# DongSky/few-shot-vit

Measured on AMD Instinct MI355X. Metric: episodes_per_sec_5way_5shot_visformer_s, higher is better.
Workload: dtype bf16; 1 GPU; BASELINE configs[1]: Visformer-S (visformer_micro_80) miniImageNet-shaped 5-way 5-shot episodic eval, 15 query/class, 80x80 fp32 NCHW episodes resident in HBM, procedural weights + calibrated BN; images_per_episode=100, encoder_chunk_images=12800, distinct_episode_batches=16, parallelism=episode-parallel x1, one all-reduce of accuracy stats, ranks_seen=1, per_rank_eps=4486.3

## Files before the change

few-shot-vit_amd/_lib.py:

```python
import ctypes as C
import os

_HERE = os.path.dirname(os.path.abspath(__file__))
LIB_PATH = os.path.join(_HERE, 'libfsvit.so')

F32, BF16, F16, BF16X2, F16X2 = 0, 1, 2, 3, 4
ACT_NONE, ACT_GELU, ACT_LRELU = 0, 1, 2
HEAD_COS, HEAD_SQR, HEAD_DOT = 0, 1, 2
ERR_ARG, ERR_KEY, ERR_IMG_SIZE, ERR_WORKSPACE = -1, -2, -3, -4


class Tensor(C.Structure):
    _fields_ = [('name', C.c_char_p), ('data', C.POINTER(C.c_float)), ('ndim', C.c_int),
                ('shape', C.c_int64 * 4)]


class VisformerCfg(C.Structure):
    _fields_ = [('img_size', C.c_int), ('init_channels', C.c_int), ('embed_dim', C.c_int),
                ('depth', C.c_int * 3), ('num_heads', C.c_int), ('mlp_ratio', C.c_float),
                ('group', C.c_int), ('bn_eps', C.c_float)]


class VitCfg(C.Structure):
    _fields_ = [('img_size', C.c_int), ('patch_size', C.c_int), ('embed_dim', C.c_int), ('depth', C.c_int),
                ('num_heads', C.c_int), ('mlp_ratio', C.c_float), ('ln_eps', C.c_float)]


class LvvitCfg(C.Structure):
    _fields_ = [('img_size', C.c_int), ('stem_channels', C.c_int), ('embed_dim', C.c_int), ('depth', C.c_int),
                ('num_heads', C.c_int), ('mlp_ratio', C.c_float), ('skip_lam', C.c_float), ('ln_eps', C.c_float),
                ('bn_eps', C.c_float)]


class ProfRec(C.Structure):
    _fields_ = [('layer', C.c_char * 48), ('kernel_id', C.c_int), ('launches', C.c_int), ('flops', C.c_double),
                ('ms', C.c_double)]


class Param(C.Structure):
    _fields_ = [('name', C.c_char_p), ('data', C.c_void_p), ('grad', C.c_void_p), ('numel', C.c_int64)]


_vp, _fp, _i, _f, _sz = C.c_void_p, C.c_void_p, C.c_int, C.c_float, C.c_size_t
SIGNATURES = {
    'fsvit_last_error': (C.c_char_p, []),
    'fsvit_version': (C.c_char_p, []),
    'fsvit_visformer_create': (_i, [C.POINTER(VisformerCfg), C.POINTER(Tensor), _i, _i, C.POINTER(_vp)]),
    'fsvit_visformer_destroy': (None, [_vp]),
    'fsvit_visformer_out_dim': (_i, [_vp]),
    'fsvit_visformer_dtype': (_i, [_vp]),
    'fsvit_visformer_workspace_bytes': (_sz, [_vp, _i]),
    'fsvit_visformer_forward': (_i, [_vp, _fp, _i, _i, _i, _fp, _vp, _sz, _vp]),
    'fsvit_vit_create': (_i, [C.POINTER(VitCfg), C.POINTER(Tensor), _i, _i, C.POINTER(_vp)]),
    'fsvit_vit_destroy': (None, [_vp]),
    'fsvit_vit_out_dim': (_i, [_vp]),
    'fsvit_vit_workspace_bytes': (_sz, [_vp, _i]),
    'fsvit_vit_forward': (_i, [_vp, _fp, _i, _i, _i, _fp, _vp, _sz, _vp]),
    'fsvit_lvvit_create': (_i, [C.POINTER(LvvitCfg), C.POINTER(Tensor), _i, _i, C.POINTER(_vp)]),
    'fsvit_lvvit_destroy': (None, [_vp]),
    'fsvit_lvvit_out_dim': (_i, [_vp]),
    'fsvit_lvvit_workspace_bytes': (_sz, [_vp, _i]),
    'fsvit_lvvit_forward': (_i, [_vp, _fp, _i, _i, _i, _fp, _vp, _sz, _vp]),
    'fsvit_lvvit_forward_map': (_i, [_vp, _fp, _i, _i, _i, _fp, _fp, _vp, _sz, _vp]),
    'fsvit_stem96_conv': (_i, [_vp, _vp, _fp, _vp, _i, _i, _vp, _i, _i, _i, _i, _i, _vp]),
    'fsvit_encoder_set_tap': (_i, [_vp, C.c_char_p, _vp, _sz]),
    'fsvit_encoder_profile_begin': (_i, [_vp]),
    'fsvit_encoder_profile_end': (_i, [_vp, C.POINTER(ProfRec), _i, C.POINTER(_i)]),
    'fsvit_kernel_name': (C.c_char_p, [_i, _i]),
    'fsvit_proto_head': (_i, [_fp, _fp, _i, _i, _i, _i, _i, _f, _i, _fp, _fp, _fp, _vp]),
    'fsvit_proto_head_devtemp': (_i, [_fp, _fp, _i, _i, _i, _i, _i, _fp, _i, _fp, _fp, _fp, _vp]),
    'fsvit_meta_baseline_forward': (_i, [_vp, _fp, _fp, _i, _i, _i, _i, _i, _i, _f, _i, _fp, _fp, _fp, _fp,
                                         _vp, _sz, _vp]),
    'fsvit_conv_gemm': (_i, [_vp, _vp, _fp, _vp, _fp, _vp] + [_i] * 15 + [_i, _vp]),
    'fsvit_conv_stem_tail': (_i, [_vp, _vp, _fp, _fp, _vp, _i, _i, _vp, _i, _i, _i, _i, _i, _i, _i, _vp]),
    'fsvit_stage1_block': (_i, [_vp, _vp, _vp, _fp, _vp, _vp, _i, _vp]),
    'fsvit_stage1_block_hw': (_i, [_vp, _vp, _vp, _fp, _vp, _vp, _i, _i, _i, _i, _vp]),
    'fsvit_visformer_last_tokens': (_i, [_vp, _vp, _sz, _i, _fp, _vp]),
    'fsvit_visformer_train_tokens': (_i, [_vp, _fp, _vp]),
    'fsvit_visformer_train_set_token_grad': (_i, [_vp, _fp]),
    'fsvit_linear_forward': (_i, [_fp, _fp, _fp, _fp, _i, _i, _i, _vp]),
    'fsvit_linear_backward': (_i, [_fp, _fp, _fp, _fp, _i, _fp, _fp, _i, _i, _i, _vp]),
    'fsvit_token_softlabel': (_i, [_fp, _fp, _i, _i, _i, _i, _i, C.c_double, _vp]),
    'fsvit_soft_target_ce': (_i, [_fp, _fp, _fp, _fp, _i, _i, _f, _vp]),
    'fsvit_row_normalize': (_i, [_fp, _fp, _fp, _i, _i, _vp]),
    'fsvit_row_normalize_backward': (_i, [_fp, _fp, _fp, _fp, _i, _i, _vp]),
    'fsvit_adamw_step': (_i, [_fp, _fp, _fp, _fp, _sz, _f, _f, _f, _f, _f, _i, _vp]),
    'fsvit_adamw_step_multi': (_i, [_vp, _i, _sz, _f, _f, _f, _f, _f, _i, _vp]),
    'fsvit_proj_mlp_rows': (_i, [_vp, _vp, _vp, _vp, _i, _i, _vp, _i, _fp, _vp, _i, _fp, _i, _i, _i, _vp]),
    'fsvit_proj_mlp_rows_dt': (_i, [_vp, _vp, _vp, _vp, _i, _i, _vp, _i, _fp, _vp, _i, _fp, _i, _i, _i, _i, _vp]),
    'fsvit_ln_linear_rows': (_i, [_vp, _vp, _vp, _i, _fp, _i, _i, _i, _f, _vp]),
    'fsvit_ln_linear_rows_dt': (_i, [_vp, _vp, _vp, _i, _fp, _i, _i, _i, _f, _i, _vp]),
    'fsvit_patch_embed2x2': (_i, [_vp, _vp, _vp, _i, _fp, _fp, _i, _i, _i, _i, _vp]),
    'fsvit_patch_embed2x2_dt': (_i, [_vp, _vp, _vp, _i, _fp, _fp, _i, _i, _i, _i, _i, _vp]),
    'fsvit_vit_block_tail': (_i, [_vp, _vp, _vp, _vp, _i, _i, _fp, _vp, _i, _fp, _vp, _i, _fp, _i, _i, _i, _f, _vp]),
    'fsvit_vit_block_tail_dt': (_i, [_vp, _vp, _vp, _vp, _i, _i, _fp, _vp, _i, _fp, _vp, _i, _fp, _i, _i, _i, _f, _i, _vp]),
    'fsvit_mlp_rows': (_i, [_vp, _vp, _vp, _i, _fp, _vp, _i, _fp, _i, _i, _i, _vp]),
    'fsvit_mlp_rows_dt': (_i, [_vp, _vp, _vp, _i, _fp, _vp, _i, _fp, _i, _i, _i, _i, _vp]),
    'fsvit_attention': (_i, [_vp, _vp, _i, _i, _i, _i, _f, _i, _vp]),
    'fsvit_op_attention_route': (_i, [_i, _i, _i]),
    'fsvit_qkv_attention': (_i, [_vp, _vp, _i, _fp, _vp, _i, _i, _i, _i, _i, _f, _vp]),
    'fsvit_qkv_attention_dt': (_i, [_vp, _vp, _i, _fp, _vp, _i, _i, _i, _i, _i, _f, _i, _vp]),
    'fsvit_vit_ln_qkv_attention': (_i, [_vp, _vp, _i, _fp, _vp, _i, _i, _i, _i, _i, _f, _f, _vp]),
    'fsvit_vit_ln_qkv_attention_dt': (_i, [_vp, _vp, _i, _fp, _vp, _i, _i, _i, _i, _i, _f, _f, _i, _vp]),
    'fsvit_im2col27': (_i, [_fp, _vp, _i, _i, _i, _i, _vp]),
    'fsvit_stem_conv1': (_i, [_fp, _vp, _i, _fp, _vp, _vp, _i, _i, _i, _vp]),
    'fsvit_stem_conv1_dt': (_i, [_fp, _vp, _i, _fp, _vp, _vp, _i, _i, _i, _i, _vp]),
    'fsvit_maxpool2_pos': (_i, [_vp, _fp, _vp, _i, _i, _i, _i, _i, _vp]),
    'fsvit_pool_affine': (_i, [_vp, _fp, _fp, _fp, _i, _i, _i, _i, _vp]),
    'fsvit_visformer_trainer_create': (_i, [C.POINTER(VisformerCfg), _i, C.POINTER(_vp)]),
    'fsvit_visformer_trainer_destroy': (None, [_vp]),
    'fsvit_visformer_trainer_workspace_bytes': (_sz, [_vp, C.POINTER(Param), _i, _i, _f]),
    'fsvit_visformer_train_forward': (_i, [_vp, C.POINTER(Param), _i, _fp, _i, _i, _i, _f, _fp, _fp, _vp, _sz, _vp]),
    'fsvit_visformer_train_backward': (_i, [_vp, C.POINTER(Param), _i, _fp, _vp]),
    'fsvit_vit_trainer_create': (_i, [C.POINTER(VitCfg), _i, C.POINTER(_vp)]),
    'fsvit_vit_trainer_destroy': (None, [_vp]),
    'fsvit_vit_trainer_droppath_calls': (_i, [_vp, _f]),
    'fsvit_vit_trainer_workspace_bytes': (_sz, [_vp, C.POINTER(Param), _i, _i, _f]),
    'fsvit_vit_train_forward': (_i, [_vp, C.POINTER(Param), _i, _fp, _i, _i, _i, _f, _fp, _fp, _vp, _sz, _vp]),
    'fsvit_vit_train_backward': (_i, [_vp, C.POINTER(Param), _i, _fp, _vp]),
    'fsvit_lvvit_trainer_create': (_i, [C.POINTER(LvvitCfg), _i, C.POINTER(_vp)]),
    'fsvit_lvvit_trainer_destroy': (None, [_vp]),
    'fsvit_lvvit_trainer_droppath_calls': (_i, [_vp, _f]),
    'fsvit_lvvit_trainer_workspace_bytes': (_sz, [_vp, C.POINTER(Param), _i, _i, _f]),
    'fsvit_lvvit_trainer_set_freeze_bn': (_i, [_vp, _i]),
    'fsvit_lvvit_train_forward': (_i, [_vp, C.POINTER(Param), _i, _fp, _i, _i, _i, _f, _fp, _fp, _vp, _sz, _vp]),
    'fsvit_lvvit_train_backward': (_i, [_vp, C.POINTER(Param), _i, _fp, _vp]),
    'fsvit_lvvit_train_tokens': (_i, [_vp, _fp, _vp]),
    'fsvit_lvvit_train_set_token_grad': (_i, [_vp, _fp]),
    'fsvit_proto_head_backward': (_i, [_fp, _fp, _fp, _i, _i, _i, _i, _i, _f, _fp, _fp, _fp, _vp]),
    'fsvit_proto_head_backward_sqr': (_i, [_fp, _fp, _fp, _i, _i, _i, _i, _i, _f, _fp, _fp, _fp, _vp]),
    'fsvit_proto_head_ce': (_i, [_fp, _fp, _vp, _i, _i, _i, _i, _i, _f, _fp, _i, _fp, _fp, _fp, _fp, _fp, _vp, _vp]),
    'fsvit_proto_head_ce_backward': (_i, [_fp, _fp, _fp, _fp, _i, _i, _i, _i, _i, _f, _fp, _i, _fp, _fp, _fp, _vp, _vp]),
    'fsvit_proto_head_backward_devtemp': (_i, [_fp, _fp, _fp, _i, _i, _i, _i, _i, _fp, _i, _fp, _fp, _fp, _vp]),
    'fsvit_visformer_trainer_set_freeze_bn': (_i, [_vp, _i]),
    'fsvit_sgd_step_multi': (_i, [_vp, _i, _sz, _f, _f, _f, _i, _vp]),
    'fsvit_sgd_step': (_i, [_fp, _fp, _fp, _sz, _f, _f, _f, _i, _vp]),
    'fsvit_sgd_nesterov_step_multi': (_i, [_vp, _i, _sz, _f, _f, _f, _i, _vp]),
    'fsvit_sgd_nesterov_step': (_i, [_fp, _fp, _fp, _sz, _f, _f, _f, _i, _vp]),
    'fsvit_grad_nan_guard_multi': (_i, [_vp, _i, _sz, _vp, _vp]),
    'fsvit_conv1x1_wgrad': (_i, [_vp, _vp, _fp, _i, _i, _i, _i, _vp]),
    'fsvit_conv3x3_wgrad': (_i, [_vp, _vp, _fp, _i, _i, _i, _i, _i, _i, _i, _vp]),
    'fsvit_gconv3x3': (_i, [_vp, _vp, _i, _vp, _i, _i, _i, _i, _vp]),
    'fsvit_image_transform_gather': (_i, [_vp, _i, _i, _vp, _i, _vp, _vp, _vp, _i, _vp, _vp, _vp, _i, _i, _i, _i, _i,
                                          C.POINTER(C.c_float), C.POINTER(C.c_float), _fp, _vp]),
    'fsvit_image_transform_rrc_gather': (_i, [_vp, _i, _i, _vp, _i, _vp, _vp, _i, _i, C.POINTER(C.c_float), C.POINTER(C.c_float), _fp, _vp]),
    'fsvit_image_transform_rrc_u8': (_i, [_vp, _i, _i, _vp, _i, _vp, _vp, _i, _i, _i, _vp, _vp]),
    'fsvit_image_strong_weak': (_i, [_vp, _i, _i, _i, _vp, _i, C.POINTER(C.c_float), C.POINTER(C.c_float), C.c_uint64, _fp, _fp, _vp]),
    'fsvit_image_rand_augment': (_i, [_vp, _i, _i, _i, _vp, _i, _vp, _i, C.POINTER(C.c_uint8), _vp]),
    'fsvit_attention_backward': (_i, [_vp, _vp, _vp, _i, _i, _i, _i, _i, _f, _i, _vp]),
    'fsvit_op_attention_bwd_route': (_i, [_i, _i, _i, _i]),
    'fsvit_op_bn_reduce_blocks': (_i, [_i]),
    'fsvit_op_ln_bwd_blocks': (_i, [_i]),
    'fsvit_op_pool_bn_bwd_blocks': (_i, [_i, _i, _i, _i, _i]),
    'fsvit_op_bn_train_forward': (_i, [_vp, _i, _i, _i, _fp, _fp, _fp, _fp, _f, _f, _i, _vp, _vp, _fp, _i, _vp, _i, _vp, _fp, _fp, _vp]),
    'fsvit_op_bn_train_backward': (_i, [_vp, _vp, _fp, _fp, _fp, _i, _i, _i, _i, _fp, _fp, _vp, _fp, _vp, _i, _vp, _fp, _fp, _fp, _fp, _vp]),
    'fsvit_op_bn_act_bwd': (_i, [_vp, _vp, _fp, _fp, _vp, _vp, _i, _i, _i, _vp]),
    'fsvit_op_stem_tail_train_forward': (_i, [_vp, _fp, _fp, _vp, _fp, _fp, _fp, _vp, _vp, _i, _i, _i, _i, _i, _vp]),
    'fsvit_op_stem_tail_train_backward': (_i, [_vp, _vp, _vp, _vp, _fp, _fp, _fp, _fp, _vp, _vp, _fp, _fp, _fp, _fp, _fp, _fp, _i, _i, _i, _i, _i, _i, _vp]),
    'fsvit_op_pool_act_bwd': (_i, [_vp, _vp, _vp, _i, _i, _i, _i, _i, _vp]),
    'fsvit_op_maxpool2_idx': (_i, [_vp, _fp, _vp, _vp, _i, _i, _i, _i, _i, _vp]),
    'fsvit_op_maxpool2_bwd': (_i, [_vp, _vp, _vp, _i, _i, _i, _i, _i, _vp]),
    'fsvit_op_ln_train_forward': (_i, [_vp, _fp, _fp, _vp, _fp, _fp, _i, _i, _f, _i, _vp]),
    'fsvit_op_ln_train_backward': (_i, [_vp, _vp, _fp, _fp, _fp, _vp, _vp, _fp, _fp, _fp, _i, _i, _i, _vp]),
    'fsvit_op_vit_assemble': (_i, [_vp, _fp, _fp, _vp, _i, _i, _i, _i, _vp]),
    'fsvit_op_vit_patch_rows': (_i, [_vp, _vp, _i, _i, _i, _i, _vp]),
    'fsvit_op_vit_cls_ln_forward': (_i, [_vp, _fp, _fp, _fp, _fp, _fp, _i, _i, _i, _f, _i, _vp]),
    'fsvit_op_vit_cls_ln_backward': (_i, [_fp, _vp, _fp, _fp, _fp, _vp, _fp, _fp, _fp, _i, _i, _i, _i, _vp]),
    'fsvit_op_vit_map_ln_forward': (_i, [_vp, _fp, _fp, _fp, _fp, _fp, _i, _i, _i, _f, _i, _vp]),
    'fsvit_op_vit_map_ln_bwd_blocks': (_i, [_i, _i]),
    'fsvit_op_vit_map_ln_backward': (_i, [_fp, _fp, _vp, _fp, _fp, _fp, _fp, _fp, _vp, _fp, _fp, _fp, _i, _i, _i, _i, _vp]),
    'fsvit_op_gelu': (_i, [_vp, _vp, _vp, _sz, _i, _vp]),
    'fsvit_op_add_scaled': (_i, [_vp, _vp, _fp, _vp, _sz, _sz, _i, _vp]),
    'fsvit_op_avgpool_bwd': (_i, [_fp, _vp, _i, _i, _i, _i, _vp]),
    'fsvit_op_batch_sum': (_i, [_vp, _fp, _i, _sz, _i, _vp]),
    'fsvit_op_bcast_add': (_i, [_vp, _fp, _vp, _i, _sz, _i, _vp]),
    'fsvit_op_colsum': (_i, [_vp, _fp, _fp, _i, _i, _i, _vp]),
    'fsvit_op_unpatch2': (_i, [_vp, _vp, _i, _i, _i, _i, _i, _vp]),
    'fsvit_op_droppath_scales': (_i, [_fp, _fp, _i, _i, C.POINTER(C.c_float), _vp]),
    'fsvit_op_fill_f32': (_i, [_fp, _f, _sz, _vp]),
    'fsvit_op_scale_copy': (_i, [_fp, _fp, _sz, _f, _vp]),
    'fsvit_op_fold_prenorm': (_i, [_fp, _fp, _fp, _vp, _fp, _i, _i, _i, _i, _vp]),
    'fsvit_op_pack_weight': (_i, [_fp, _vp] + [_i] * 13 + [_vp]),
    'fsvit_op_pack_weight_multi': (_i, [C.POINTER(_fp), C.POINTER(_vp), C.POINTER(_i), _i, _i, _vp]),
    'fsvit_op_conv_train': (_i, [_vp, _vp, _fp, _vp, _vp, _vp] + [_i] * 15 + [C.POINTER(_i), _vp]),
    'fsvit_op_gconv3x3_train': (_i, [_vp, _vp, _i, _vp, _vp, _vp, _i, _i, _i, _i, _vp]),
    'fsvit_op_stage1_block_train': (_i, [_vp, _vp, _vp, _fp, _vp, _i, _vp, _vp, _vp, _vp, _vp, _vp, _fp, _fp, _fp, _i, _i, _i, _i, _vp]),
    'fsvit_op_stage1_block_dgrad': (_i, [_vp, _vp, _vp, _vp, _i, _vp, _vp, _vp, _vp, _vp, _i, _i, _i, _i, _vp]),
    'fsvit_emd_head_workspace_bytes': (_sz, [_i, _i, _i, _i, _i]),
    'fsvit_emd_head_forward': (_i, [_fp, _fp, _i, _i, _i, _i, _i, _f, _fp, _fp, _vp, _vp, _sz, _vp]),
# ... 47 lines not shown
```

few-shot-vit_amd/csrc/conv3x3_halo.hip:

```cpp
#include <stdlib.h>

#include <type_traits>

#include "conv_gemm.h"
#include "lds_dma.h"

namespace FSVIT_NS {

__device__ __attribute__((aligned(256))) unsigned char g_zero_page_halo[256];
#define HWAIT(vm) asm volatile("s_waitcnt vmcnt(" #vm ") lgkmcnt(0)" ::: "memory")

template <int CTRL>
__device__ __forceinline__ float quad_xor(float v) {
  return __builtin_bit_cast(float, __builtin_amdgcn_update_dpp(0, __builtin_bit_cast(int, v), CTRL, 0xf, 0xf, true));
}

namespace halo {
constexpr int TR = 8, TW = 40;
constexpr int HR = TR + 2, HP = 44;
constexpr int PLANE = 7168;
constexpr int NPIECE = 7;
constexpr int HBUF = 8 * PLANE;
constexpr int NST = 3, STAGE = 16384;
constexpr int OFF_W = 2 * HBUF;
constexpr int LDS_BYTES = OFF_W + NST * STAGE;
static_assert(LDS_BYTES == 160 * 1024, "the two halo buffers and the weight ring fill the LDS exactly");
}

template <int CIN, bool FUSE_TAIL, bool STATS = false, int CREAL = CIN>
__global__ __launch_bounds__(512, 2) void conv3x3_halo_kernel(const ConvGemmParams p, const int n_tiles) {
  using namespace halo;
  extern __shared__ __attribute__((aligned(16))) unsigned char smem[];
  constexpr int NH = CIN / 64;
  constexpr int NKM = 9 * NH, NKT = NKM + (FUSE_TAIL ? 1 : 0);
  constexpr int MT = 5, NT = 4;
  const int t = threadIdx.x, lane = t & 63;
  const int wave = __builtin_amdgcn_readfirstlane(t >> 6);
  const int wm = wave >> 1, wn = wave & 1;
  const int lrow = lane & 15, lq = lane >> 4;
  const unsigned lds0 = lds_addr(smem);
  unsigned char* const wst0 = smem + OFF_W;

  const unsigned char* const Xb = reinterpret_cast<const unsigned char*>(p.x);
  const unsigned char* const Wb = reinterpret_cast<const unsigned char*>(p.w);
  bf16* __restrict__ Y = reinterpret_cast<bf16*>(p.y);
  const int tiles_per_img = p.H / TR;

  const int fr = ((lrow >> 3) & 1) * 2 + ((lrow >> 1) & 1), fc = ((lrow >> 2) & 1) * 2 + (lrow & 1);
  auto blk_r = [&](int i) { return (wm * MT + i) / (TW / 4); };
  auto blk_c = [&](int i) { return (wm * MT + i) % (TW / 4); };
  f32x4 st0[STATS ? NT : 1], st1[STATS ? NT : 1];
#pragma unroll
  for (int j = 0; j < (STATS ? NT : 1); ++j) st0[j] = st1[j] = f32x4{0.f, 0.f, 0.f, 0.f};
  unsigned xb[MT];
#pragma unroll
  for (int i = 0; i < MT; ++i) xb[i] = (unsigned)(((blk_r(i) * 4 + fr) * HP + blk_c(i) * 4 + fc) * 16 + lq * PLANE);
  const int srow = lane >> 3;
  const unsigned schunk = (unsigned)(((lane & 7) ^ srow) << 4);
  unsigned offB[2];
#pragma unroll
  for (int j = 0; j < 2; ++j) {
    const int R = (2 * wave + j) * 8 + srow;
    const int ch = (R & ~31) + 8 * ((R & 15) >> 2) + 4 * ((R >> 4) & 1) + (R & 3);
    offB[j] = (unsigned)ch * (unsigned)(p.Kw * 2) + schunk;
  }
  const unsigned b_rd = (unsigned)((wn * 64 + lrow) * 128);
  const unsigned sw0 = (unsigned)((lq ^ (lrow & 7)) << 4), sw1 = (unsigned)(((4 + lq) ^ (lrow & 7)) << 4);

  auto issue_w = [&](int wk, int stage) {
    const unsigned d = lds0 + OFF_W + stage * STAGE;
    dma2(offB[0], offB[1], Wb + (size_t)wk * 128, d + (2 * wave) * 1024, d + (2 * wave + 1) * 1024);
  };
  const int x_rs = p.x_planar ? (CIN / 8) * p.W * 16 : p.W * CREAL * 2, x_ps = p.x_planar ? 16 : CREAL * 2;
  auto issue_piece = [&](int j, int lane_o, const unsigned char* base, bool top, bool bot, int nb) {
    const int s = j * 64 + lane_o, hr = s / HP, hc = s - hr * HP;
    const bool ok = (base != nullptr) & (s < HR * HP) & (hc >= 1) & (hc <= TW) & !(top & (hr == 0)) & !(bot & (hr == HR - 1));
    const unsigned long a = (unsigned long)base + (unsigned long)(unsigned)(hr * x_rs + (hc - 1) * x_ps);
    const unsigned long z = (unsigned long)g_zero_page_halo;
    dma1_lane(reinterpret_cast<const void*>(ok ? a : z), lds0 + nb * HBUF + wave * PLANE + j * 1024);
  };
  auto halo_base = [&](int tile, int h) {
    const int bb = tile / tiles_per_img, rr = (tile - bb * tiles_per_img) * TR;
    if constexpr (CREAL != CIN) {
      if (h * 64 + wave * 8 >= CREAL) return (const unsigned char*)nullptr;
    }
    return Xb + (long)(bb * p.H + rr - 1) * x_rs + (p.x_planar ? (h * 8 + wave) * p.W * 16 : h * 128 + wave * 16);
  };

  f32x4 acc[MT][NT];
#pragma unroll
  for (int i = 0; i < MT; ++i)
#pragma unroll
    for (int j = 0; j < NT; ++j) acc[i][j] = f32x4{0.f, 0.f, 0.f, 0.f};

  int tix = blockIdx.x;
  if (tix >= n_tiles) return;
  const int my_tiles = (n_tiles - tix + (int)gridDim.x - 1) / (int)gridDim.x;
  int steps_left = my_tiles * NKT;

  auto wk_of = [&](int q) { return q >= NKM ? NKM : (NH == 2 ? (q >= 9 ? (q - 9) * 2 + 1 : q * 2) : q); };

  {
    const int r00 = (tix % tiles_per_img) * TR;
    const unsigned char* b0 = halo_base(tix, 0);
#pragma unroll
    for (int j = 0; j < NPIECE; ++j) issue_piece(j, lane, b0, r00 == 0, r00 + TR == p.H, 0);
  }
  issue_w(wk_of(0), 0);
  issue_w(wk_of(1 % NKT), 1);
  HWAIT(0);
  bar();
  int st_cur = 0, st_pre = 2, q_pre = 2 % NKT;
  int buf = 0;
#define H_STAMP(acc_)

  auto advance = [&]() {
    st_cur = st_cur == NST - 1 ? 0 : st_cur + 1;
    st_pre = st_pre == NST - 1 ? 0 : st_pre + 1;
    q_pre = q_pre == NKT - 1 ? 0 : q_pre + 1;
    --steps_left;
  };

  while (true) {
    const int tnext = tix + (int)gridDim.x;
    const bool has_next = tnext < n_tiles;
    const int b = tix / tiles_per_img, r0 = (tix - b * tiles_per_img) * TR;
    u32x4 xf0[MT], wf0[NT];

#pragma unroll 1
    for (int h = 0; h < NH; ++h) {
      const int n_tix = h + 1 < NH ? tix : (has_next ? tnext : -1), n_h = h + 1 < NH ? h + 1 : 0;
      const unsigned char* nbase = n_tix >= 0 ? halo_base(n_tix, n_h) : nullptr;
      const int n_r0 = n_tix >= 0 ? (n_tix % tiles_per_img) * TR : 0;
      const bool n_top = n_r0 == 0, n_bot = n_r0 + TR == p.H;
      int lane_o = lane;
      asm volatile("" : "+v"(lane_o));
      u32x4 xf1[MT], wf1[NT];
      {
        const unsigned char* wb = wst0 + st_cur * STAGE + b_rd;
#pragma unroll
        for (int j = 0; j < NT; ++j) wf0[j] = *reinterpret_cast<const u32x4*>(wb + j * 2048 + sw0);
#pragma unroll
        for (int i = 0; i < MT; ++i) xf0[i] = *reinterpret_cast<const u32x4*>(smem + xb[i]);
      }
      H_STAMP(ckP);
      static_for<9>([&](auto tapc) {
        constexpr int TAP = decltype(tapc)::value;
        constexpr int TOFF = ((TAP / 3) * HP + TAP % 3) * 16;
        constexpr int TOFF_N = (((TAP + 1) / 3) * HP + (TAP + 1) % 3) * 16;
        const bool pre_w = steps_left > 2;
        if (pre_w) issue_w(wk_of(q_pre), st_pre);
        __builtin_amdgcn_sched_barrier(0);
        {
          const unsigned char* wb = wst0 + st_cur * STAGE + b_rd;
#pragma unroll
          for (int j = 0; j < NT; ++j) wf1[j] = *reinterpret_cast<const u32x4*>(wb + j * 2048 + sw1);
#pragma unroll
          for (int i = 0; i < MT; ++i) xf1[i] = *reinterpret_cast<const u32x4*>(smem + xb[i] + 4 * PLANE + TOFF);
        }
#pragma unroll
        for (int i = 0; i < MT; ++i)
#pragma unroll
          for (int j = 0; j < NT; ++j) acc[i][j] = mma_chunk<bf16>(wf0[j], xf0[i], acc[i][j]);
#pragma unroll
        for (int k = 0; k < MT + NT; ++k) {
          __builtin_amdgcn_sched_group_barrier(0x008, 1, 0);
          __builtin_amdgcn_sched_group_barrier(0x100, 1, 0);
        }
        __builtin_amdgcn_sched_group_barrier(0x008, MT * NT - (MT + NT), 0);
        __builtin_amdgcn_sched_barrier(0);
        H_STAMP(ckA);
        if (TAP >= 1 && TAP <= NPIECE) { if (pre_w) HWAIT(3); else HWAIT(1); }
        else { if (pre_w) HWAIT(2); else HWAIT(0); }
        H_STAMP(ckV);
        bar();
        H_STAMP(ckW);
        if constexpr (TAP < NPIECE) issue_piece(TAP, lane_o, nbase, n_top, n_bot, buf ^ 1);
        const int st_next = st_cur == NST - 1 ? 0 : st_cur + 1;
        if constexpr (TAP < 8) {
          const unsigned char* wb = wst0 + st_next * STAGE + b_rd;
#pragma unroll
          for (int j = 0; j < NT; ++j) wf0[j] = *reinterpret_cast<const u32x4*>(wb + j * 2048 + sw0);
#pragma unroll
          for (int i = 0; i < MT; ++i) xf0[i] = *reinterpret_cast<const u32x4*>(smem + xb[i] + TOFF_N);
        } else if (FUSE_TAIL) {
          if (h == NH - 1) {
            const bf16* X2 = reinterpret_cast<const bf16*>(p.x2);
#pragma unroll
            for (int i = 0; i < MT; ++i) {
              const int lr = lane_o & 15;
              const int fr_o = ((lr >> 3) & 1) * 2 + ((lr >> 1) & 1), fc_o = ((lr >> 2) & 1) * 2 + (lr & 1);
              const size_t pix = (size_t)(b * p.H + r0 + blk_r(i) * 4 + fr_o) * p.W + blk_c(i) * 4 + fc_o;
              xf0[i] = gload16(X2 + pix * p.x2_cstride + lq * 8);
            }
          }
        }
#pragma unroll
        for (int i = 0; i < MT; ++i)
#pragma unroll
          for (int j = 0; j < NT; ++j) acc[i][j] = mma_chunk<bf16>(wf1[j], xf1[i], acc[i][j]);
        if constexpr (TAP < NPIECE) {
#pragma unroll
          for (int k = 0; k < 8; ++k) {
            __builtin_amdgcn_sched_group_barrier(0x008, 1, 0);
            __builtin_amdgcn_sched_group_barrier(0x002, 3, 0);
          }
#pragma unroll
// ... 98 lines not shown
                  if (posrow && n < CREAL) v[u] += *reinterpret_cast<const f32x4*>(posrow + n + 4 * u);
                } else v[u] += *reinterpret_cast<const f32x4*>(posrow + n + 4 * u);
              }
            }
            bool nst = true;
            if constexpr (CREAL != CIN) nst = n < CREAL;
            if (nst && (!FUSE_TAIL || (lrow_e & 3) == 0)) {
              const bf16x8 o = {(bf16)v[0][0], (bf16)v[0][1], (bf16)v[0][2], (bf16)v[0][3], (bf16)v[1][0], (bf16)v[1][1], (bf16)v[1][2], (bf16)v[1][3]};
              if (!FUSE_TAIL && p.y_planar) *reinterpret_cast<bf16x8*>(Y + (((size_t)(b * p.H + r0 + prow_i) * (p.y_cstride >> 3) + (n >> 3)) * p.W + pcol_i) * 8) = o;
              else *reinterpret_cast<bf16x8*>(Y + orow * p.y_cstride + n) = o;
            }
          }
        }
      };
      auto finish_pooled = [&](auto actf) {
        const int u_e = lrow_e & 3;
        const int nq = wn * 64 + (u_e >> 1) * 32 + lq_e * 8 + (u_e & 1) * 4;
        bool qok = true;
        if constexpr (CREAL != CIN) qok = nq < CREAL;
        const f32x4 bq = (p.bias && qok) ? *reinterpret_cast<const f32x4*>(p.bias + nq) : f32x4{0.f, 0.f, 0.f, 0.f};
        const int ph = p.H >> 1, pw = p.W >> 1;
#pragma unroll
        for (int i = 0; i < MT; ++i) {
          const int py = (r0 + blk_r(i) * 4 + fr_e) >> 1, px = (blk_c(i) * 4 + fc_e) >> 1;
          f32x4 pq;
          if constexpr (CREAL != CIN) pq = (p.pos && qok) ? *reinterpret_cast<const f32x4*>(p.pos + (size_t)(py * pw + px) * p.y_cstride + nq) : f32x4{0.f, 0.f, 0.f, 0.f};
          else pq = *reinterpret_cast<const f32x4*>(p.pos + (size_t)(py * pw + px) * p.y_cstride + nq);
          f32x4 m[NT];
#pragma unroll
          for (int j = 0; j < NT; ++j) {
            m[j] = acc[i][j];
            acc[i][j] = f32x4{0.f, 0.f, 0.f, 0.f};
#pragma unroll
            for (int e = 0; e < 4; ++e) {
              m[j][e] = fmaxf(m[j][e], quad_xor<0xB1>(m[j][e]));
              m[j][e] = fmaxf(m[j][e], quad_xor<0x4E>(m[j][e]));
            }
          }
          f32x4 v = u_e == 0 ? m[0] : (u_e == 1 ? m[1] : (u_e == 2 ? m[2] : m[3]));
          v += bq;
#pragma unroll
          for (int e = 0; e < 4; ++e) v[e] = actf(v[e]);
          v += pq;
          if (qok) store4<bf16>(Y + ((size_t)(b * ph + py) * pw + px) * p.y_cstride + nq, v);
        }
      };
      if (FUSE_TAIL && p.act == ACT_LRELU) finish_pooled([](float x) { return fmaxf(x, 0.1f * x); });
      else if (FUSE_TAIL && p.act == ACT_NONE) finish_pooled([](float x) { return x; });
      else if (p.act == ACT_GELU) finish([](float x) { return gelu_sig(x); });
      else if (p.act == ACT_LRELU) finish([](float x) { return fmaxf(x, 0.1f * x); });
      else finish([](float x) { return x; });
    }
    H_STAMP(ckE);
    if (!has_next) break;
    tix = tnext;
  }
  asm volatile("s_waitcnt vmcnt(0)" ::: "memory");
  if constexpr (STATS) {
    __syncthreads();
    float* red = reinterpret_cast<float*>(smem);
#pragma unroll
    for (int j = 0; j < NT; ++j)
#pragma unroll
      for (int e = 0; e < 4; ++e) {
        float a = st0[j][e], q = st1[j][e];
#pragma unroll
        for (int o = 1; o < 16; o <<= 1) { a += __shfl_xor(a, o); q += __shfl_xor(q, o); }
        if (lrow == 0) {
          const int cl = (j >> 1) * 32 + lq * 8 + (j & 1) * 4 + e;
          red[(wave * 2 + 0) * 64 + cl] = a;
          red[(wave * 2 + 1) * 64 + cl] = q;
        }
      }
    __syncthreads();
    if (t < 256) {
      const int which = t >> 7, c = t & 127, h = c >> 6, cl = c & 63;
      float a = 0.f;
#pragma unroll
      for (int m = 0; m < 4; ++m) a += red[((m * 2 + h) * 2 + which) * 64 + cl];
      p.stats[((size_t)blockIdx.x * 2 + which) * p.y_cstride + c] = a;
    }
  }
}

bool conv3x3_halo_eligible(const ConvGemmParams& p, int dtype) {
  if (dtype != 1) return false;
  if (p.KH != 3 || p.KW != 3 || p.stride != 1 || p.pad != 1 || p.groups != 1) return false;
  if (p.w_cpad) {
    if (p.w_cpad != 128 || p.Cin != 96 || p.N != 96 || p.x_cstride != 96 || p.y_cstride != 96 || p.K != 9 * 96) return false;
    if (p.W != halo::TW || (p.H % halo::TR) || p.OH != p.H || p.OW != p.W) return false;
    if (p.res || p.y2 || p.act == ACT_MUL || p.act == ACT_GELU || p.y_rpi || p.out_f32 || p.w_rstride || p.w_gstride || p.stats || p.x_planar || p.y_planar) return false;
    if (p.pool2) return p.x2 && p.K2 == 32 && p.x2_cstride >= 32 && p.Kw == 9 * 128 + 64;
    return !p.x2 && !p.pos && p.Kw == 9 * 128;
  }
  if (p.N != 128 || p.y_cstride != 128 || p.W != halo::TW || (p.H % halo::TR) || p.OH != p.H || p.OW != p.W) return false;
  if (p.res || p.y2 || p.act == ACT_MUL || p.y_rpi || p.out_f32 || p.w_rstride || p.w_gstride) return false;
  if (p.Cin != p.x_cstride || p.K != 9 * p.Cin) return false;
  if (p.stats && (p.pool2 || p.act != ACT_NONE)) return false;
  if (p.y_planar && (p.pool2 || p.stats)) return false;
  if (p.pool2) return p.Cin == 128 && p.x2 && p.K2 == 32 && p.x2_cstride >= 32 && p.pos && p.Kw == p.K + 64;
  return (p.Cin == 64 || p.Cin == 128) && !p.x2 && !p.pos && p.Kw == p.K;
}

static inline int halo_grid(const ConvGemmParams& p) { const int n_tiles = p.B * (p.H / halo::TR); return n_tiles < 256 ? n_tiles : 256; }
int conv3x3_halo_stats_rows(const ConvGemmParams& p, int dtype) {
  ConvGemmParams q = p;
  float dummy;
  q.stats = &dummy;
  return conv3x3_halo_eligible(q, dtype) ? halo_grid(p) : 0;
}

template <int CIN, bool FUSE_TAIL, bool STATS = false, int CREAL = CIN>
static int launch_halo_t(const ConvGemmParams& p, hipStream_t stream) {
  const int n_tiles = p.B * (p.H / halo::TR);
  auto kern = conv3x3_halo_kernel<CIN, FUSE_TAIL, STATS, CREAL>;
  hipError_t e = hipFuncSetAttribute((const void*)kern, hipFuncAttributeMaxDynamicSharedMemorySize, halo::LDS_BYTES);
  if (e != hipSuccess) return (int)e;
  const int grid = n_tiles < 256 ? n_tiles : 256;
  hipLaunchKernelGGL(kern, dim3(grid), dim3(512), halo::LDS_BYTES, stream, p, n_tiles);
  return (int)hipGetLastError();
}

int launch_conv3x3_halo(const ConvGemmParams& p, hipStream_t stream) {
  if (p.w_cpad) return p.pool2 ? launch_halo_t<128, true, false, 96>(p, stream) : launch_halo_t<128, false, false, 96>(p, stream);
  if (p.pool2) return launch_halo_t<128, true>(p, stream);
  if (p.stats) return p.Cin == 64 ? launch_halo_t<64, false, true>(p, stream) : launch_halo_t<128, false, true>(p, stream);
  return p.Cin == 64 ? launch_halo_t<64, false>(p, stream) : launch_halo_t<128, false>(p, stream);
}

}
```

few-shot-vit_amd/csrc/engine.hip:

```cpp
#include "../../include/fsvit.h"

#include <hip/hip_runtime.h>

#include <cmath>
#include <cstdarg>
#include <cstdio>
#include <cstring>
#include <cstdlib>
#include <utility>
#include <cstdint>
#include <initializer_list>
#include <map>
#include <string>
#include <vector>

#include "kernels.h"
#include "train_kernels.h"

using namespace fsvit;

#define K(fn) ((kdt == FSVIT_F16 || kdt == FSVIT_F16X2) ? fsvit_f16::fn : fsvit::fn)
static inline bool is_x2(int dtype) { return dtype == FSVIT_BF16X2 || dtype == FSVIT_F16X2; }
static inline bool known_dtype(int dtype) { return dtype >= FSVIT_F32 && dtype <= FSVIT_F16X2; }
static inline int kd(int dtype) { return (dtype == FSVIT_F32 || is_x2(dtype)) ? 0 : 1; }
// ... 226 lines not shown
  }
  for (int y = 0; y < k; ++y) for (int x = 0; x < k; ++x) f[(size_t)y * k + x] = f1[y] * f1[x];
  return f;
}

inline double gelu_exact(double z) { return 0.5 * z * (1.0 + std::erf(z * 0.7071067811865476)); }

void gauss_moments_gelu(double mu, double sig, double* mean, double* var) {
  double sw = 0, s1 = 0, s2 = 0;
  for (int j = 0; j <= 256; ++j) {
    const double z = -8.0 + j / 16.0, w = std::exp(-0.5 * z * z), v = gelu_exact(mu + sig * z);
    sw += w; s1 += w * v; s2 += w * v * v;
  }
  *mean = s1 / sw;
  *var = std::max(0.0, s2 / sw - (s1 / sw) * (s1 / sw));
}

double lrelu_mean(double mu, double sig) {
  if (sig <= 0) return mu > 0 ? mu : 0.1 * mu;
  const double t = mu / sig;
  return mu * (0.1 + 0.9 * 0.5 * (1.0 + std::erf(t * 0.7071067811865476))) + 0.9 * sig * std::exp(-0.5 * t * t) * 0.3989422804014327;
}

int pack_layer(EngineBase* h, Layer* L, const float* W, int O, int Ig, int KH, int KW, int groups,
               const std::vector<double>* out_scale, const std::vector<double>* in_scale,
               const std::vector<double>& bias, bool has_bias,
               const std::vector<int>* rowmap, int Npad, const std::vector<int>* colmap, int Kpad,
               const WRound* wr = nullptr, const std::vector<double>* in_mean = nullptr, const double* tapf = nullptr,
               bool use_cst = false, std::vector<double>* corr_out = nullptr) {
  const int bke = 128 / h->es;
  const int N = (rowmap ? Npad : O) / groups;
  const int K = colmap ? Kpad : KH * KW * Ig;
  const int Kw = round_up(K, bke);
  const bool fix = wr && wr->on && in_mean && in_mean->size() >= (size_t)groups * Ig;
  const bool cst = wr && wr->on && use_cst && wr->cst.size() >= (size_t)groups * Ig;
  if (corr_out) corr_out->assign(O, 0.0);
  std::vector<float> pk((size_t)groups * N * Kw, 0.0f);
  std::vector<float> pb((size_t)groups * N, 0.0f);
  for (int o = 0; o < O; ++o) {
    const int row = rowmap ? (*rowmap)[o] : o;
    const double so = out_scale ? (*out_scale)[o] : 1.0;
    const int g0 = (o / (O / groups)) * Ig;
    double corr = 0.0, wc = 0.0;
    for (int c = 0; c < Ig; ++c) {
      const double si = in_scale ? (*in_scale)[c] : 1.0;
      for (int ky = 0; ky < KH; ++ky)
        for (int kx = 0; kx < KW; ++kx) {
          int k = (ky * KW + kx) * Ig + c;
          if (colmap) k = (*colmap)[k];
          const double v = (double)W[(((size_t)o * Ig + c) * KH + ky) * KW + kx] * so * si;
          pk[(size_t)row * Kw + k] = (float)v;
          if (fix) corr -= (wr->rounded(v) - v) * (tapf ? tapf[ky * KW + kx] : 1.0) * (*in_mean)[g0 + c];
          if (cst) wc += v * wr->cst[g0 + c];
        }
    }
    if (has_bias) pb[row] = (float)(bias[o] + corr + wc);
    else if (corr_out) (*corr_out)[o] = corr;
  }
  L->N = N; L->K = K; L->Kw = Kw; L->groups = groups;
  RC_TRY(upload(h, pk, true, &L->w));
  if (has_bias) { void* b; RC_TRY(upload(h, pb, false, &b)); L->bias = (float*)b; }
  return 0;
}

std::vector<double> prenorm_bias(const float* W, int O, int C, const std::vector<double>& t) {
  std::vector<double> b(O, 0.0);
  for (int o = 0; o < O; ++o) {
    double s = 0.0;
    for (int c = 0; c < C; ++c) s += (double)W[(size_t)o * C + c] * t[c];
    b[o] = s;
  }
  return b;
}

int pack_pos(EngineBase* h, const float* pos, int C, int HW, float** out) {
  std::vector<float> p((size_t)HW * C);
  for (int c = 0; c < C; ++c)
    for (int i = 0; i < HW; ++i) p[(size_t)i * C + c] = pos[(size_t)c * HW + i];
  void* d; RC_TRY(upload(h, p, false, &d));
  *out = (float*)d;
  return 0;
}

int build(fsvit_visformer* h, const SD& sd) {
  const int kdt = h->dtype;
  const fsvit_visformer_cfg& cf = h->cfg;
  const double eps = cf.bn_eps;
  const int epc = 16 / h->es;
  const int D = cf.embed_dim;
  h->C0 = cf.init_channels; h->C1 = D / 2; h->C2 = D; h->C3 = h->out_dim = D * 2;
  if (cf.img_size % 16 != 0) return fail(FSVIT_ERR_ARG, "img_size %d must be a multiple of 16", cf.img_size);
  h->H0 = cf.img_size / 2; h->H1 = cf.img_size / 4; h->H2 = cf.img_size / 8; h->H3 = cf.img_size / 16;
  if (cf.group < 2) return fail(FSVIT_ERR_ARG, "group < 2 ('net' setting, visformer.py:137-138) is not supported");
  h->hid1 = h->C1 * 2;
  h->hid2 = (int)(h->C2 * cf.mlp_ratio);
  h->hid3 = (int)(h->C3 * cf.mlp_ratio);
  h->hd2 = (int)std::lround((double)(h->C2 / cf.num_heads));
  h->hd3 = (int)std::lround((double)(h->C3 / cf.num_heads));
  h->hdp2 = K(attention_padded_head_dim)(h->hd2, h->H2 * h->H2, kd(kdt));
  h->hdp3 = K(attention_padded_head_dim)(h->hd3, h->H3 * h->H3, kd(kdt));
  const int Cg = h->hid1 / cf.group;
  if (h->C0 % epc || h->C1 % epc || h->hid1 % cf.group || Cg % epc)
    return fail(FSVIT_ERR_ARG, "channel counts must be multiples of %d for 16-byte K chunks", epc);
  if (!is_pow2(h->C0) || !is_pow2(h->C1) || !is_pow2(h->C2) || !is_pow2(Cg))
    return fail(FSVIT_ERR_ARG, "multi-tap conv input channels must be powers of two");
  if (h->H2 * h->H2 > 128) return fail(FSVIT_ERR_ARG, "attention supports at most 128 tokens (img_size <= 88)");

  std::vector<double> nob;
  WRound wr;
  const char* wr_env = getenv("FSVIT_WROUND");
  wr.on = (kdt == FSVIT_BF16 || kdt == FSVIT_F16) && !(wr_env && wr_env[0] == '0');
  wr.f16 = kdt == FSVIT_F16;
  if (wr.on) wr.cst.assign(h->C1, 0.0);
  auto vec = [&](const std::string& name, int C, bool absolute) {
    const float* p = sd.get(name, {C});
    std::vector<double> v(C, 0.0);
    for (int c = 0; p && c < C; ++c) v[c] = absolute ? std::fabs((double)p[c]) : (double)p[c];
    return v;
  };
  {
    const float* w1 = sd.get("stem.conv1.weight", {h->C0, 3, 3, 3});
    const float* wd = sd.get("stem.downsample.0.weight", {h->C1, 3, 3, 3});
    const float* w2 = sd.get("stem.conv2.weight", {h->C1, h->C0, 3, 3});
    const float* w3 = sd.get("stem.conv3.weight", {h->C1, h->C1, 3, 3});
    Affine b1 = bn_affine(sd, "stem.bn1", h->C0, eps), b2 = bn_affine(sd, "stem.bn2", h->C1, eps);
    Affine b3 = bn_affine(sd, "stem.bn3", h->C1, eps), bd = bn_affine(sd, "stem.downsample.1", h->C1, eps);
    if (!w1 || !wd || !w2 || !w3 || !b1.ok || !b2.ok || !b3.ok || !bd.ok) return FSVIT_ERR_KEY;
    std::vector<int> cm(27);
    for (int k = 0; k < 27; ++k) cm[k] = k;
    std::vector<double> m2(h->C0), m3(h->C1);
    {
      const std::vector<double> be1 = vec("stem.bn1.bias", h->C0, false), ga1 = vec("stem.bn1.weight", h->C0, true);
      const std::vector<double> be2 = vec("stem.bn2.bias", h->C1, false), ga2 = vec("stem.bn2.weight", h->C1, true);
      for (int c = 0; c < h->C0; ++c) m2[c] = lrelu_mean(be1[c], ga1[c]);
      for (int c = 0; c < h->C1; ++c) m3[c] = lrelu_mean(be2[c], ga2[c]);
    }
    const std::vector<double> tf0 = tap_fraction(h->H0, 1, 3, 1);
    RC_TRY(pack_layer(h, &h->conv1, w1, h->C0, 3, 3, 3, 1, &b1.s, nullptr, b1.t, true, nullptr, 0, &cm, 32));
    RC_TRY(pack_layer(h, &h->conv2, w2, h->C1, h->C0, 3, 3, 1, &b2.s, nullptr, b2.t, true, nullptr, 0, nullptr, 0, &wr, &m2, tf0.data()));
    {
      const int bke = 128 / h->es, K = 9 * h->C1, Kmain = round_up(K, bke), Kw = Kmain + bke;
      std::vector<float> pk((size_t)h->C1 * Kw, 0.0f), pb(h->C1);
      for (int o = 0; o < h->C1; ++o) {
        double corr = 0.0;
        for (int c = 0; c < h->C1; ++c)
          for (int t9 = 0; t9 < 9; ++t9) {
            const double v = (double)w3[((size_t)o * h->C1 + c) * 9 + t9] * b3.s[o];
            pk[(size_t)o * Kw + t9 * h->C1 + c] = (float)v;
            if (wr.on) corr -= (wr.rounded(v) - v) * tf0[t9] * m3[c];
          }
        for (int c = 0; c < 3; ++c)
          for (int t9 = 0; t9 < 9; ++t9)
            pk[(size_t)o * Kw + Kmain + t9 * 3 + c] = (float)((double)wd[((size_t)o * 3 + c) * 9 + t9] * bd.s[o]);
        pb[o] = (float)(b3.t[o] + bd.t[o] + corr);
      }
      h->conv3f.N = h->C1; h->conv3f.K = K; h->conv3f.Kw = Kw; h->conv3f.groups = 1;
      RC_TRY(upload(h, pk, true, &h->conv3f.w));
      void* bdev; RC_TRY(upload(h, pb, false, &bdev)); h->conv3f.bias = (float*)bdev;
    }
  }
  {
    const float* p1 = sd.get("pos_embed1", {1, h->C1, h->H1, h->H1});
    const float* p2 = sd.get("pos_embed2", {1, h->C2, h->H2, h->H2});
    const float* p3 = sd.get("pos_embed3", {1, h->C3, h->H3, h->H3});
    if (!p1 || !p2 || !p3) return FSVIT_ERR_KEY;
    RC_TRY(pack_pos(h, p1, h->C1, h->H1 * h->H1, &h->pos1));
    RC_TRY(pack_pos(h, p2, h->C2, h->H2 * h->H2, &h->pos2));
    RC_TRY(pack_pos(h, p3, h->C3, h->H3 * h->H3, &h->pos3));
  }
  std::vector<double> x_mean(h->C1, 0.0);
  h->s1.resize(cf.depth[0]);
  for (int i = 0; i < cf.depth[0]; ++i) {
    const std::string p = "stage1." + std::to_string(i) + ".";
    Affine n2 = bn_affine(sd, p + "norm2.bn", h->C1, eps);
    const float* w1 = sd.get(p + "mlp.conv1.weight", {h->hid1, h->C1, 1, 1});
    const float* w2 = sd.get(p + "mlp.conv2.weight", {h->hid1, Cg, 3, 3});
    const float* w3 = sd.get(p + "mlp.conv3.weight", {h->C1, h->hid1, 1, 1});
    if (!n2.ok || !w1 || !w2 || !w3) return FSVIT_ERR_KEY;
    const std::vector<double> rm = vec(p + "norm2.bn.running_mean", h->C1, false);
    std::vector<double> mh2(h->hid1, 0.0), corr3;
    if (wr.on) {
      if (wr.cst.empty()) wr.cst.assign(h->C1, 0.0);
      const std::vector<double> be = vec(p + "norm2.bn.bias", h->C1, false), ga = vec(p + "norm2.bn.weight", h->C1, true);
      const std::vector<double> tf1 = tap_fraction(h->H1, 1, 3, 1);
      std::vector<double> mh1(h->hid1), vh1(h->hid1);
      for (int n = 0; n < h->hid1; ++n) {
        double mu = 0, var = 0;
        for (int c = 0; c < h->C1; ++c) { const double w = w1[(size_t)n * h->C1 + c]; mu += w * be[c]; var += w * w * ga[c] * ga[c]; }
        gauss_moments_gelu(mu, std::sqrt(var), &mh1[n], &vh1[n]);
// ... 63 lines not shown
    blocks.resize(cf.depth[s - 1]);
    std::vector<int> rowmap(3 * heads * hd), colmap(heads * hd);
    for (int x = 0; x < 3; ++x)
      for (int y = 0; y < heads; ++y)
        for (int z = 0; z < hd; ++z) rowmap[(x * heads + y) * hd + z] = (x * heads + y) * hdp + z;
    for (int y = 0; y < heads; ++y)
      for (int z = 0; z < hd; ++z) colmap[y * hd + z] = y * hdp + z;
    for (int i = 0; i < cf.depth[s - 1]; ++i) {
      const std::string p = "stage" + std::to_string(s) + "." + std::to_string(i) + ".";
      Affine n1 = bn_affine(sd, p + "norm1.bn", C, eps), n2 = bn_affine(sd, p + "norm2.bn", C, eps);
      const float* wq = sd.get(p + "attn.qkv.weight", {3 * heads * hd, C, 1, 1});
      const float* wp = sd.get(p + "attn.proj.weight", {C, heads * hd, 1, 1});
      const float* w1 = sd.get(p + "mlp.conv1.weight", {hid, C, 1, 1});
      const float* w3 = sd.get(p + "mlp.conv3.weight", {C, hid, 1, 1});
      if (!n1.ok || !n2.ok || !wq || !wp || !w1 || !w3) return FSVIT_ERR_KEY;
      const std::vector<double> rm1 = vec(p + "norm1.bn.running_mean", C, false), rm2 = vec(p + "norm2.bn.running_mean", C, false);
      std::vector<double> mctx(heads * hd, 0.0), mh(hid, 0.0), corr_p, corr_3;
      if (wr.on) {
        const std::vector<double> be1 = vec(p + "norm1.bn.bias", C, false);
        const std::vector<double> be2 = vec(p + "norm2.bn.bias", C, false), ga2 = vec(p + "norm2.bn.weight", C, true);
        for (int n = 0; n < heads * hd; ++n) {
          double a = 0;
          for (int c = 0; c < C; ++c) a += (double)wq[((size_t)2 * heads * hd + n) * C + c] * be1[c];
          mctx[n] = a;
        }
        for (int n = 0; n < hid; ++n) {
          double mu = 0, var = 0, dummy;
          for (int c = 0; c < C; ++c) { const double w = w1[(size_t)n * C + c]; mu += w * be2[c]; var += w * w * ga2[c] * ga2[c]; }
          gauss_moments_gelu(mu, std::sqrt(var), &mh[n], &dummy);
        }
      }
      RC_TRY(pack_layer(h, &blocks[i].qkv, wq, 3 * heads * hd, C, 1, 1, 1, nullptr, &n1.s, prenorm_bias(wq, 3 * heads * hd, C, n1.t), true, &rowmap, 3 * heads * hdp, nullptr, 0,
                        &wr, &rm1, nullptr, true));
      RC_TRY(pack_layer(h, &blocks[i].proj, wp, C, heads * hd, 1, 1, 1, nullptr, nullptr, nob, false, nullptr, 0, &colmap, heads * hdp, &wr, &mctx, nullptr, false, &corr_p));
      if (wr.on) for (int o = 0; o < C; ++o) wr.cst[o] += corr_p[o];
      RC_TRY(pack_layer(h, &blocks[i].fc1, w1, hid, C, 1, 1, 1, nullptr, &n2.s, prenorm_bias(w1, hid, C, n2.t), true, nullptr, 0, nullptr, 0, &wr, &rm2, nullptr, true));
      RC_TRY(pack_layer(h, &blocks[i].fc2, w3, C, hid, 1, 1, 1, nullptr, nullptr, nob, false, nullptr, 0, nullptr, 0, &wr, &mh, nullptr, false, &corr_3));
      if (wr.on) {
        x_mean.assign(C, 0.0);
        for (int o = 0; o < C; ++o) {
          double a = rm2[o];
          for (int c = 0; c < hid; ++c) a += (double)w3[(size_t)o * hid + c] * mh[c];
          x_mean[o] = a;
          wr.cst[o] += corr_3[o];
        }
      }
      if (K(mlp_rows_supported)(kd(kdt), C, hid)) {
        const int kc = K(mlp_rows_proj_supported)(C, hid, heads * hdp) ? heads * hdp : 0;
        BlockA& b = blocks[i];
        void* b1i = nullptr;
        RC_TRY(packed_image(h, K(mlp_rows_image_bytes)(C, hid, kc), &b.mlp_img, [&](void* img) {
          HIP_TRY(hipMalloc(&b1i, (size_t)hid * 4));
          h->allocs.push_back(b1i);
          return K(launch_mlp_pack)(b.fc1.w, b.fc1.Kw, b.fc1.bias, b.fc2.w, b.fc2.Kw, b.proj.w, b.proj.Kw, kc, img, (float*)b1i, C, hid, nullptr);
        }));
        b.mlp_b1 = (float*)b1i;
        b.mlp_kc = kc;
      }
      if (K(qkv_attn_supported)(kd(kdt), C, heads, hdp, (s == 2 ? h->H2 : h->H3) * (s == 2 ? h->H2 : h->H3))) {
        RC_TRY(packed_image(h, K(qkv_attn_image_bytes)(), &blocks[i].qa_img,
                            [&](void* img) { return K(launch_qkv_attn_pack)(blocks[i].qkv.w, blocks[i].qkv.Kw, img, nullptr); }));
      } else if (K(qkv_attn_rows_supported)(kd(kdt), C, heads, hdp, (s == 2 ? h->H2 : h->H3) * (s == 2 ? h->H2 : h->H3))) {
        RC_TRY(packed_image(h, K(ln_gemm_rows_image_bytes)(C, 3 * heads * hdp), &blocks[i].qar_img,
                            [&](void* img) { return K(launch_qkv_attn_rows_pack)(blocks[i].qkv.w, blocks[i].qkv.Kw, img, C, heads, hdp, nullptr); }));
      } else if (K(gemm_rows_supported)(kd(kdt), C, 3 * heads * hdp)) {
        RC_TRY(packed_image(h, K(ln_gemm_rows_image_bytes)(C, 3 * heads * hdp), &blocks[i].qr_img,
                            [&](void* img) { return K(launch_ln_gemm_pack)(blocks[i].qkv.w, blocks[i].qkv.Kw, img, C, 3 * heads * hdp, nullptr); }));
      }
    }
  }
  {
    Affine bn = bn_affine(sd, "norm.bn", h->C3, eps);
    if (!bn.ok) return FSVIT_ERR_KEY;
    std::vector<float> s(h->C3), t(h->C3);
    for (int c = 0; c < h->C3; ++c) { s[c] = (float)bn.s[c]; t[c] = (float)(bn.t[c] + (wr.on ? bn.s[c] * wr.cst[c] : 0.0)); }
    void* d; RC_TRY(upload(h, s, false, &d)); h->fscale = (float*)d;
    RC_TRY(upload(h, t, false, &d)); h->fshift = (float*)d;
  }
  return 0;
}

struct Plan {
  size_t patches, c1, c2;
  size_t ha, hb;
  size_t qkv, ctx, hid;
  size_t x1, x1b, x2, x3;
  size_t total;
};

size_t align256(size_t v) { return (v + 255) / 256 * 256; }

Plan make_plan(const fsvit_visformer* h, size_t Bc) {
  Plan p;
  const size_t es = h->es, P0 = (size_t)h->H0 * h->H0, P1 = (size_t)h->H1 * h->H1, P2 = (size_t)h->H2 * h->H2, P3 = (size_t)h->H3 * h->H3;
  const int heads = h->cfg.num_heads;
  size_t off = 0;
  auto take = [&](size_t bytes) { size_t o = off; off += align256(bytes); return o; };
  p.x1 = take(Bc * P1 * h->C1 * es);
  p.x1b = take(Bc * P1 * h->C1 * es);
  p.x2 = take(Bc * P2 * h->C2 * es);
  p.x3 = take(Bc * P3 * h->C3 * es);
  const size_t scratch0 = off;
  p.patches = take(Bc * P0 * 32 * es);
  p.c1 = take(Bc * P0 * h->C0 * es);
  p.c2 = take(Bc * P0 * h->C1 * es);
  size_t hi = off;
  off = scratch0;
  p.ha = take(Bc * P1 * h->hid1 * es);
  p.hb = take(Bc * P1 * h->hid1 * es);
  if (off > hi) hi = off;
  off = scratch0;
  size_t q2 = Bc * P2 * 3 * heads * h->hdp2 * es, q3 = Bc * P3 * 3 * heads * h->hdp3 * es;
  size_t c2 = Bc * P2 * heads * h->hdp2 * es, c3 = Bc * P3 * heads * h->hdp3 * es;
  size_t h2 = Bc * P2 * h->hid2 * es, h3 = Bc * P3 * h->hid3 * es;
  p.qkv = take(q2 > q3 ? q2 : q3);
  p.ctx = take(c2 > c3 ? c2 : c3);
  p.hid = take(h2 > h3 ? h2 : h3);
  if (off > hi) hi = off;
  p.total = hi;
  return p;
}

ConvGemmParams conv_params(const Layer& L, const void* x, void* y, int B, int H, int W, int Cin, int x_cstride,
                           int KH, int KW, int stride, int pad, int y_cstride, int act,
                           const void* res, int res_first, const float* pos) {
  ConvGemmParams p;
  p.x = x; p.w = L.w; p.bias = L.bias; p.res = res; p.pos = pos; p.y = y;
  p.B = B; p.H = H; p.W = W; p.Cin = Cin; p.x_cstride = x_cstride;
  p.OH = (H + 2 * pad - KH) / stride + 1; p.OW = (W + 2 * pad - KW) / stride + 1;
  p.KH = KH; p.KW = KW; p.stride = stride; p.pad = pad;
  p.N = L.N; p.y_cstride = y_cstride; p.K = L.K; p.Kw = L.Kw; p.M = B * p.OH * p.OW;
  p.groups = L.groups; p.act = act; p.res_first = res_first; p.log2Cin = ilog2(Cin);
  p.x2 = nullptr; p.x2_cstride = 0; p.K2 = 0; p.pool2 = 0; p.y_rpi = 0; p.y_row0 = 0;
  p.w_gstride = 0; p.w_rstride = 0; p.out_f32 = 0; p.y2 = nullptr; p.stats = nullptr;
  return p;
}

int tap(EngineBase* h, const std::string& name, const void* src, size_t bytes, bool first, hipStream_t st) {
  if (!first || h->taps.empty()) return 0;
  auto it = h->taps.find(name);
  if (it == h->taps.end() || it->second.dst == nullptr) return 0;
  size_t n = bytes < it->second.bytes ? bytes : it->second.bytes;
  HIP_TRY(hipMemcpyAsync(it->second.dst, src, n, hipMemcpyDeviceToDevice, st));
  return 0;
}

enum { KID_GEMM256 = 0, KID_GEMM64 = 1, KID_GEMM32 = 2, KID_IM2COL = 3, KID_MAXPOOL = 4, KID_ATTN = 5, KID_POOL = 6, KID_HEAD = 7, KID_STAGE1 = 8, KID_GEMM128 = 9, KID_HALO = 12, KID_MLPROWS = 13, KID_QKVATTN = 15, KID_STEMCONV1 = 16, KID_GCONV_X2 = 14, KID_STAGE1RING = 17, KID_LNGEMM = 18, KID_QKVATTNROWS = 19, KID_VITATTNROWS = 20 };


template <typename F>
int timed(EngineBase* h, hipStream_t st, const char* layer, int kernel, double flops, F&& launch) {
  if (!h->profiling) return launch();
  hipEvent_t e0 = h->prof_last, e1;
  if (!e0) { HIP_TRY(hipEventCreate(&e0)); HIP_TRY(hipEventRecord(e0, st)); }
  int rc = launch();
  if (rc != 0) return rc;
  HIP_TRY(hipEventCreate(&e1));
  HIP_TRY(hipEventRecord(e1, st));
  h->prof.push_back(ProfEntry{layer, kernel, flops, e0, e1});
  h->prof_last = e1;
  return 0;
}

static constexpr int stem_slice_images() { return 3200; }

int run_gemm(EngineBase* h, hipStream_t st, const char* layer, const Layer& L, const ConvGemmParams& p, double n_true, double k_true) {
  const int kdt = h->dtype;
  const double flops = 2.0 * (double)p.M * n_true * k_true * (double)p.groups;
  static const int kid_of_cfg[4] = {KID_GEMM256, KID_GEMM64, KID_GEMM32, KID_GEMM128};
  const int route = K(conv_gemm_route)(p, kg(kdt));
  const int kid = route == 0 ? KID_HALO : route == 1 ? KID_GEMM256 : route == 3 ? KID_GCONV_X2 : kid_of_cfg[K(conv_gemm_v2_config)(p)];
  return timed(h, st, layer, kid, flops, [&]() { return K(launch_conv_gemm)(p, kg(kdt), st); });
}

int forward_chunk(fsvit_visformer* h, const float* x, int Bc, float* feat, unsigned char* ws, bool first, hipStream_t st,
                  const float* xsrc2 = nullptr, int B1 = 0) {
  const Plan pl = make_plan(h, Bc);
  const int kdt = h->dtype, dt = kd(kdt);
  const size_t es = h->es;
  const int heads = h->cfg.num_heads;
  void *patches = ws + pl.patches, *c1 = ws + pl.c1, *c2 = ws + pl.c2;
  void *x1 = ws + pl.x1, *x1b = ws + pl.x1b, *x2 = ws + pl.x2, *x3 = ws + pl.x3, *ha = ws + pl.ha, *hb = ws + pl.hb;
  void *qkv = ws + pl.qkv, *ctx = ws + pl.ctx, *hid = ws + pl.hid;
  const int img = h->cfg.img_size;

  h->prof_last = nullptr;
  if (!xsrc2) B1 = Bc;
  const bool conv1_fused = K(stem_conv1_supported)(dt, img, h->C0);
  ConvGemmParams p2 = conv_params(h->conv2, c1, c2, Bc, h->H0, h->H0, h->C0, h->C0, 3, 3, 1, 1, h->C1, ACT_LRELU, nullptr, 0, nullptr);
  ConvGemmParams p3 = conv_params(h->conv3f, c2, x1, Bc, h->H0, h->H0, h->C1, h->C1, 3, 3, 1, 1, h->C1, ACT_LRELU, nullptr, 0, h->pos1);
  p3.x2 = patches; p3.x2_cstride = 32; p3.K2 = 32; p3.pool2 = 1;
  const bool planar = conv1_fused && K(conv_gemm_route)(p2, kg(kdt)) == 0 && K(conv_gemm_route)(p3, kg(kdt)) == 0;
  p2.x_planar = p2.y_planar = p3.x_planar = planar ? 1 : 0;
  if (planar) {
    const int S = stem_slice_images();
    const size_t s_pat = (size_t)h->H0 * h->H0 * 32 * es, s_c1 = (size_t)h->H0 * h->H0 * h->C0 * es, s_c2 = (size_t)h->H0 * h->H0 * h->C1 * es,
                 s_x1 = (size_t)h->H1 * h->H1 * h->C1 * es;
    const double fl1 = 2.0 * 27.0 * h->C0 * h->H0 * h->H0;
    for (int g0 = 0; g0 < Bc; g0 += S) {
      const int g1 = g0 + S < Bc ? g0 + S : Bc;
      for (int part = 0; part < 2; ++part) {
        const int a = part == 0 ? g0 : (g0 > B1 ? g0 : B1), b = part == 0 ? (g1 < B1 ? g1 : B1) : g1;
        if (a >= b) continue;
        const float* src = part == 0 ? x + (size_t)a * 3 * img * img : xsrc2 + (size_t)(a - B1) * 3 * img * img;
        RC_TRY(timed(h, st, "stem.im2col+conv1", KID_STEMCONV1, fl1 * (b - a), [&]() {
          return K(launch_stem_conv1)(src, (unsigned char*)patches + a * s_pat, (unsigned char*)c1 + a * s_c1, h->conv1.w, h->conv1.Kw, h->conv1.bias, b - a, st, 1); }));
      }
      ConvGemmParams q2 = p2, q3 = p3;
      q2.x = (const unsigned char*)c1 + g0 * s_c1; q2.y = (unsigned char*)c2 + g0 * s_c2; q2.B = g1 - g0; q2.M = (g1 - g0) * q2.OH * q2.OW;
      q3.x = (const unsigned char*)c2 + g0 * s_c2; q3.x2 = (const unsigned char*)patches + g0 * s_pat; q3.y = (unsigned char*)x1 + g0 * s_x1;
      q3.B = g1 - g0; q3.M = (g1 - g0) * q3.OH * q3.OW;
      RC_TRY(run_gemm(h, st, "stem.conv2", h->conv2, q2, h->C1, 9.0 * h->C0));
      RC_TRY(run_gemm(h, st, "stem.conv3+down+pool", h->conv3f, q3, h->C1, 9.0 * h->C1 + 27.0));
    }
  } else {
    if (conv1_fused) {
      const double fl1 = 2.0 * 27.0 * h->C0 * h->H0 * h->H0;
      RC_TRY(timed(h, st, "stem.im2col+conv1", KID_STEMCONV1, fl1 * B1, [&]() {
        return K(launch_stem_conv1)(x, patches, c1, h->conv1.w, h->conv1.Kw, h->conv1.bias, B1, st, 0); }));
      if (Bc > B1)
        RC_TRY(timed(h, st, "stem.im2col+conv1", KID_STEMCONV1, fl1 * (Bc - B1), [&]() {
          return K(launch_stem_conv1)(xsrc2, (unsigned char*)patches + (size_t)B1 * h->H0 * h->H0 * 32 * es, (unsigned char*)c1 + (size_t)B1 * h->H0 * h->H0 * h->C0 * es,
                                   h->conv1.w, h->conv1.Kw, h->conv1.bias, Bc - B1, st, 0); }));
    } else {
      RC_TRY(timed(h, st, "stem.im2col", KID_IM2COL, 0.0, [&]() { return K(launch_im2col27)(x, patches, B1, img, img, h->H0, h->H0, dt, st); }));
      if (Bc > B1)
        RC_TRY(timed(h, st, "stem.im2col", KID_IM2COL, 0.0, [&]() {
          return K(launch_im2col27)(xsrc2, (unsigned char*)patches + (size_t)B1 * h->H0 * h->H0 * 32 * es, Bc - B1, img, img, h->H0, h->H0, dt, st); }));
      RC_TRY(run_gemm(h, st, "stem.conv1", h->conv1, conv_params(h->conv1, patches, c1, Bc, h->H0, h->H0, 32, 32, 1, 1, 1, 0, h->C0, ACT_LRELU, nullptr, 0, nullptr), h->C0, 27));
    }
    RC_TRY(run_gemm(h, st, "stem.conv2", h->conv2, p2, h->C1, 9.0 * h->C0));
    RC_TRY(run_gemm(h, st, "stem.conv3+down+pool", h->conv3f, p3, h->C1, 9.0 * h->C1 + 27.0));
  }
  RC_TRY(tap(h, "stem", x1, (size_t)Bc * h->H1 * h->H1 * h->C1 * es, first, st));

  const int Cg = h->hid1 / h->cfg.group;
  const bool fuse1 = K(stage1_ring_supported)(dt, h->C1, h->hid1, h->cfg.group, h->H1) && h->s1.size() && h->s1[0].c2.Kw == 320;
  for (size_t i = 0; i < h->s1.size(); ++i) {
    const Block1& b = h->s1[i];
    if (fuse1) {
      const double fl = 2.0 * Bc * h->H1 * h->H1 * ((double)h->hid1 * h->C1 + (double)h->hid1 * 9 * Cg + (double)h->C1 * h->hid1);
      RC_TRY(timed(h, st, "stage1.block", KID_STAGE1RING, fl,
                   [&]() { return K(launch_stage1_ring)(x1, x1b, b.c1.w, b.c1.bias, b.c2.w, b.c3.w, Bc, h->H1, h->H1, st, b.c3s); }));
      std::swap(x1, x1b);
    } else {
      RC_TRY(run_gemm(h, st, "stage1.mlp.conv1", b.c1, conv_params(b.c1, x1, ha, Bc, h->H1, h->H1, h->C1, h->C1, 1, 1, 1, 0, h->hid1, ACT_GELU, nullptr, 0, nullptr), h->hid1, h->C1));
      RC_TRY(run_gemm(h, st, "stage1.mlp.conv2", b.c2, conv_params(b.c2, ha, hb, Bc, h->H1, h->H1, Cg, h->hid1, 3, 3, 1, 1, h->hid1, ACT_GELU, nullptr, 0, nullptr), Cg, 9.0 * Cg));
      RC_TRY(run_gemm(h, st, "stage1.mlp.conv3", b.c3, conv_params(b.c3, hb, x1, Bc, h->H1, h->H1, h->hid1, h->hid1, 1, 1, 1, 0, h->C1, ACT_NONE, x1, 0, nullptr), h->C1, h->hid1));
    }
    RC_TRY(tap(h, "stage1." + std::to_string(i), x1, (size_t)Bc * h->H1 * h->H1 * h->C1 * es, first, st));
  }

  for (int s = 2; s <= 3; ++s) {
    const int Ci = s == 2 ? h->C1 : h->C2, C = s == 2 ? h->C2 : h->C3;
    const int Hi = s == 2 ? h->H1 : h->H2, Ho = s == 2 ? h->H2 : h->H3;
    const int hidc = s == 2 ? h->hid2 : h->hid3, hd = s == 2 ? h->hd2 : h->hd3, hdp = s == 2 ? h->hdp2 : h->hdp3;
    void* xin = s == 2 ? x1 : x2;
    void* xs = s == 2 ? x2 : x3;
    const Layer& pe = s == 2 ? h->pe2 : h->pe3;
    const float* pos = s == 2 ? h->pos2 : h->pos3;
    const size_t xbytes = (size_t)Bc * Ho * Ho * C * es;
    const std::string sp = "stage" + std::to_string(s);
    if (h->pe_img[s - 2]) {
      RC_TRY(timed(h, st, s == 2 ? "patch_embed2" : "patch_embed3", KID_LNGEMM, 2.0 * Bc * Ho * Ho * 4.0 * Ci * C,
                   [&]() { return K(launch_patch_embed_rows)(xin, xs, h->pe_img[s - 2], pe.bias, pos, Bc, Hi, Ci, C, st); }));
    } else
    RC_TRY(run_gemm(h, st, s == 2 ? "patch_embed2" : "patch_embed3", pe, conv_params(pe, xin, xs, Bc, Hi, Hi, Ci, Ci, 2, 2, 2, 0, C, ACT_NONE, nullptr, 0, pos), C, 4.0 * Ci));
    RC_TRY(tap(h, "patch_embed" + std::to_string(s), xs, xbytes, first, st));
    const std::vector<BlockA>& blocks = s == 2 ? h->s2 : h->s3;
    const float scale = 1.0f / std::sqrt((float)hd);
    const int S = Ho * Ho;
    for (size_t i = 0; i < blocks.size(); ++i) {
      const BlockA& b = blocks[i];
      if (b.qa_img) {
        RC_TRY(timed(h, st, (sp + ".attn.qkv+core").c_str(), KID_QKVATTN, 2.0 * Bc * S * (3.0 * heads * hd) * C + 4.0 * Bc * heads * (double)S * S * hd,
                     [&]() { return K(launch_qkv_attn)(xs, ctx, b.qa_img, b.qkv.bias, Bc, S, scale, st); }));
      } else if (b.qar_img) {
        RC_TRY(timed(h, st, (sp + ".attn.qkv+core").c_str(), KID_QKVATTNROWS, 2.0 * Bc * S * (3.0 * heads * hd) * C + 4.0 * Bc * heads * (double)S * S * hd,
                     [&]() { return K(launch_qkv_attn_rows)(xs, ctx, b.qar_img, b.qkv.bias, Bc, S, C, heads, hdp, scale, st); }));
      } else {
      if (b.qr_img) {
        RC_TRY(timed(h, st, (sp + ".attn.qkv").c_str(), KID_LNGEMM, 2.0 * Bc * S * (3.0 * heads * hd) * C,
// ... 17 lines not shown
        RC_TRY(run_gemm(h, st, (sp + ".mlp.conv1").c_str(), b.fc1, conv_params(b.fc1, xs, hid, Bc, Ho, Ho, C, C, 1, 1, 1, 0, hidc, ACT_GELU, nullptr, 0, nullptr), hidc, C));
        RC_TRY(run_gemm(h, st, (sp + ".mlp.conv3").c_str(), b.fc2, conv_params(b.fc2, hid, xs, Bc, Ho, Ho, hidc, hidc, 1, 1, 1, 0, C, ACT_NONE, xs, 0, nullptr), C, hidc));
      }
      RC_TRY(tap(h, sp + "." + std::to_string(i), xs, xbytes, first, st));
    }
  }
  RC_TRY(timed(h, st, "norm.pool", KID_POOL, 0.0, [&]() { return K(launch_pool_affine)(x3, h->fscale, h->fshift, feat, Bc, h->H3 * h->H3, h->C3, dt, st); }));
  return 0;
}

size_t visformer_plan_bytes(const EngineBase* h, size_t Bc) { return make_plan(static_cast<const fsvit_visformer*>(h), Bc).total; }
int visformer_chunk(EngineBase* h, const float* x, int Bc, float* feat, unsigned char* ws, bool first, hipStream_t st) {
  return forward_chunk(static_cast<fsvit_visformer*>(h), x, Bc, feat, ws, first, st);
}

template <class H>
void encoder_destroy(H* h) {
  if (!h) return;
  for (void* p : h->allocs) (void)hipFree(p);
  delete h;
}

template <class H, class Cfg>
int encoder_create(const Cfg* cfg, const fsvit_tensor* state_dict, int n_tensors, int dtype, H** out, bool bad_cfg, const char* bad_cfg_msg, int kind,
                   int (*build_fn)(H*, const SD&), size_t (*plan_bytes)(const EngineBase*, size_t),
                   int (*chunk)(EngineBase*, const float*, int, float*, unsigned char*, bool, hipStream_t), const char* size_fmt) {
  if (!cfg || !state_dict || !out || n_tensors <= 0) return fail(FSVIT_ERR_ARG, "null argument");
  if (!known_dtype(dtype)) return fail(FSVIT_ERR_ARG, "unknown dtype %d", dtype);
  if (bad_cfg) return fail(FSVIT_ERR_ARG, "%s", bad_cfg_msg);
  H* h = new H();
  h->kind = kind;
  h->cfg = *cfg;
  h->img_size = cfg->img_size;
  h->dtype = dtype;
  h->es = storage_bytes(dtype);
  h->plan_bytes = plan_bytes; h->chunk = chunk; h->size_fmt = size_fmt;
  SD sd{state_dict, n_tensors};
  int rc = build_fn(h, sd);
  if (rc != 0) { encoder_destroy(h); return rc; }
  *out = h;
  return 0;
}

size_t encoder_workspace_bytes(const EngineBase* h, int chunk_images) {
  if (!h || chunk_images <= 0) return 0;
  return h->plan_bytes(h, (size_t)chunk_images);
}

const char* const SIZE_FMT_VISFORMER = "Input image size (%d*%d) does not match model (%d*%d).";
const char* const SIZE_FMT_VIT = "Input image size (%d*%d) doesn't match model (%d*%d).";

int encoder_forward(EngineBase* h, const float* x, int n_img, int img_h, int img_w, float* feat, void* ws, size_t ws_bytes, void* stream) {
  if (h && n_img <= 0) return 0;
  if (!h || !x || !feat || !ws) return fail(FSVIT_ERR_ARG, "null argument");
  if (img_h != h->img_size || img_w != h->img_size) return fail(FSVIT_ERR_IMG_SIZE, h->size_fmt, img_h, img_w, h->img_size, h->img_size);
  if (((uintptr_t)ws & 255) != 0) return fail(FSVIT_ERR_ARG, "workspace must be 256-byte aligned");
  int lo = 0, hi = n_img;
  while (lo < hi) {
    int mid = (lo + hi + 1) / 2;
    if (h->plan_bytes(h, (size_t)mid) <= ws_bytes) lo = mid; else hi = mid - 1;
  }
  if (lo < 1) return fail(FSVIT_ERR_WORKSPACE, "workspace of %zu bytes cannot hold one image (need %zu)", ws_bytes, h->plan_bytes(h, 1));
  const size_t img_elems = (size_t)3 * img_h * img_w;
  for (int off = 0; off < n_img; off += lo) {
    const int bc = n_img - off < lo ? n_img - off : lo;
    int rc = h->chunk(h, x + (size_t)off * img_elems, bc, feat + (size_t)off * h->out_dim, (unsigned char*)ws, off == 0, (hipStream_t)stream);
    if (rc != 0) return rc;
  }
  return 0;
}

}

extern "C" int fsvit_visformer_create(const fsvit_visformer_cfg* cfg, const fsvit_tensor* state_dict, int n_tensors,
                                      int dtype, fsvit_visformer** out) {
  const bool bad = cfg && (cfg->num_heads < 1 || cfg->embed_dim < 2 || cfg->init_channels < 1 || cfg->depth[0] < 0 || cfg->depth[1] < 0 || cfg->depth[2] < 0);
  return encoder_create(cfg, state_dict, n_tensors, dtype, out, bad, "bad Visformer configuration", KIND_VISFORMER, build, visformer_plan_bytes, visformer_chunk,
                        SIZE_FMT_VISFORMER);
}
extern "C" void fsvit_visformer_destroy(fsvit_visformer* h) { encoder_destroy(h); }
extern "C" int fsvit_visformer_out_dim(const fsvit_visformer* h) { return h ? h->out_dim : 0; }
extern "C" int fsvit_visformer_dtype(const fsvit_visformer* h) { return h ? h->dtype : -1; }
extern "C" size_t fsvit_visformer_workspace_bytes(const fsvit_visformer* h, int chunk_images) { return encoder_workspace_bytes(h, chunk_images); }

extern "C" int fsvit_encoder_set_tap(void* hv, const char* name, void* dst_dev, size_t bytes) {
  EngineBase* h = static_cast<EngineBase*>(hv);
  if (!h || !name) return fail(FSVIT_ERR_ARG, "null argument");
  if (!dst_dev) h->taps.erase(name);
  else h->taps[name] = Tap{dst_dev, bytes};
  return 0;
}

extern "C" int fsvit_visformer_forward(fsvit_visformer* h, const float* x, int n_img, int img_h, int img_w,
                                       float* feat, void* ws, size_t ws_bytes, void* stream) {
  return encoder_forward(h, x, n_img, img_h, img_w, feat, ws, ws_bytes, stream);
}

extern "C" int fsvit_visformer_last_tokens(fsvit_visformer* h, const void* ws, size_t ws_bytes, int n_img, float* tokens, void* stream) {
  const int kdt = h ? h->dtype : FSVIT_BF16;
  if (!h || !ws || !tokens || n_img <= 0) return fail(FSVIT_ERR_ARG, "bad argument");
  const Plan pl = make_plan(h, (size_t)n_img);
  if (pl.total > ws_bytes) return fail(FSVIT_ERR_WORKSPACE, "last_tokens: the forward of %d images did not fit one chunk of this workspace", n_img);
  RC_TRY(K(launch_tokens_to_f32)((const unsigned char*)ws + pl.x3, h->fscale, h->fshift, tokens, (size_t)n_img * h->H3 * h->H3 * h->C3, h->C3, kd(kdt),
                              (hipStream_t)stream));
  return 0;
}

extern "C" int fsvit_proto_head(const float* fs, const float* fq, int E, int way, int shot, int Q, int D, float temp,
                                int method, float* logits, float* acc, float* loss, void* stream) {
  if (!fs || !fq || !logits) return fail(FSVIT_ERR_ARG, "null argument");
  if (method != FSVIT_HEAD_COS && method != FSVIT_HEAD_SQR && method != FSVIT_HEAD_DOT) return fail(FSVIT_ERR_ARG, "unknown head method %d", method);
  RC_TRY(fsvit::launch_proto_head(fs, fq, E, way, shot, Q, D, temp, method, logits, acc, loss, (hipStream_t)stream, nullptr));
  return 0;
}

extern "C" int fsvit_proto_head_devtemp(const float* fs, const float* fq, int E, int way, int shot, int Q, int D, const float* temp_dev,
                                        int method, float* logits, float* acc, float* loss, void* stream) {
  if (!fs || !fq || !logits || !temp_dev) return fail(FSVIT_ERR_ARG, "null argument");
  if (method != FSVIT_HEAD_COS && method != FSVIT_HEAD_SQR && method != FSVIT_HEAD_DOT) return fail(FSVIT_ERR_ARG, "unknown head method %d", method);
  RC_TRY(fsvit::launch_proto_head(fs, fq, E, way, shot, Q, D, 0.f, method, logits, acc, loss, (hipStream_t)stream, temp_dev));
  return 0;
}

extern "C" int fsvit_meta_baseline_forward(void* hv, const float* x_shot, const float* x_query, int E, int way,
                                           int shot, int Q, int img_h, int img_w, float temp, int method, float* logits,
                                           float* acc, float* loss, float* feat, void* ws, size_t ws_bytes, void* stream) {
  if (!hv || !feat) return fail(FSVIT_ERR_ARG, "null argument");
  EngineBase* eb = static_cast<EngineBase*>(hv);
  if (!eb->chunk) return fail(FSVIT_ERR_ARG, "not an fsvit encoder handle");
  const int ns = E * way * shot, nq = E * Q, D = eb->out_dim;
  {
    if (eb->kind == KIND_VISFORMER && x_shot && x_query && ns > 0 && nq > 0) {
      fsvit_visformer* h = static_cast<fsvit_visformer*>(eb);
      if (img_h != h->cfg.img_size || img_w != h->cfg.img_size)
        return fail(FSVIT_ERR_IMG_SIZE, SIZE_FMT_VISFORMER, img_h, img_w, h->cfg.img_size, h->cfg.img_size);
      if (ws && ((uintptr_t)ws & 255) == 0 && make_plan(h, (size_t)ns + nq).total <= ws_bytes) {
        int rc1 = forward_chunk(h, x_shot, ns + nq, feat, (unsigned char*)ws, true, (hipStream_t)stream, x_query, ns);
        if (rc1 != 0) return rc1;
        return fsvit_proto_head(feat, feat + (size_t)ns * D, E, way, shot, Q, D, temp, method, logits, acc, loss, stream);
      }
    }
  }
  int rc = encoder_forward(eb, x_shot, ns, img_h, img_w, feat, ws, ws_bytes, stream);
  if (rc != 0) return rc;
  rc = encoder_forward(eb, x_query, nq, img_h, img_w, feat + (size_t)ns * D, ws, ws_bytes, stream);
  if (rc != 0) return rc;
  return fsvit_proto_head(feat, feat + (size_t)ns * D, E, way, shot, Q, D, temp, method, logits, acc, loss, stream);
}

extern "C" int fsvit_conv_gemm(const void* x, const void* w, const float* bias, const void* res, const float* pos, void* y,
                               int B, int H, int W, int Cin, int x_cstride, int KH, int KW, int stride, int pad, int N,
                               int y_cstride, int Kw, int groups, int act, int res_first, int dtype, void* stream) {
  const int kdt = dtype;
  if (!known_dtype(dtype)) return fail(FSVIT_ERR_ARG, "unknown dtype %d", dtype);
  if (!x || !w || !y) return fail(FSVIT_ERR_ARG, "null argument");
  const int es = storage_bytes(dtype), epc = 16 / es, bke = 128 / es;
  if (Cin % epc || x_cstride % epc || N % 4 || y_cstride % 4 || Kw % bke || Kw < KH * KW * Cin)
    return fail(FSVIT_ERR_ARG, "conv_gemm alignment: Cin/x_cstride %% %d, N/y_cstride %% 4, Kw %% %d", epc, bke);
  if (KH * KW > 1 && !is_pow2(Cin) && Cin % 32) return fail(FSVIT_ERR_ARG, "multi-tap conv needs a power-of-two Cin or a multiple of 32");
  Layer L; L.w = const_cast<void*>(w); L.bias = const_cast<float*>(bias); L.N = N; L.K = KH * KW * Cin; L.Kw = Kw; L.groups = groups;
  ConvGemmParams p = conv_params(L, x, y, B, H, W, Cin, x_cstride, KH, KW, stride, pad, y_cstride, act, res, res_first, pos);
  RC_TRY(K(launch_conv_gemm)(p, kg(dtype), (hipStream_t)stream));
  return 0;
}

extern "C" int fsvit_conv_stem_tail(const void* x, const void* w, const float* bias, const float* pos, const void* x2, int x2_cstride, int K2,
// ... 234 lines not shown
  void* img = nullptr;
  if (C == 512) {
    if (!K(qkv_attn_rows_supported)(1, C, heads, hdp, S) || kw < C)
      return fail(FSVIT_ERR_ARG, "fsvit_qkv_attention: C = 512 needs head dim 96 (padded) and S <= 32");
    HIP_TRY(hipMalloc(&img, K(ln_gemm_rows_image_bytes)(C, 3 * heads * hdp)));
    int rc = K(launch_qkv_attn_rows_pack)(wqkv, kw, img, C, heads, hdp, st);
    if (rc == 0) rc = K(launch_qkv_attn_rows)(x, ctx, img, bias, B, S, C, heads, hdp, scale, st);
    (void)hipStreamSynchronize(st);
    (void)hipFree(img);
    if (rc != 0) return hipfail((hipError_t)rc, "fsvit_qkv_attention");
    return 0;
  }
  if (!K(qkv_attn_supported)(1, C, heads, hdp, S) || kw < C)
    return fail(FSVIT_ERR_ARG, "fsvit_qkv_attention: only C = 256, 6 heads x 48 (padded), S <= 112 is built");
  HIP_TRY(hipMalloc(&img, K(qkv_attn_image_bytes)()));
  int rc = K(launch_qkv_attn_pack)(wqkv, kw, img, st);
  if (rc == 0) rc = K(launch_qkv_attn)(x, ctx, img, bias, B, S, scale, st);
  (void)hipStreamSynchronize(st);
  (void)hipFree(img);
  if (rc != 0) return hipfail((hipError_t)rc, "fsvit_qkv_attention");
  return 0;
}

extern "C" int fsvit_vit_ln_qkv_attention(const void* x, const void* wqkv, int kw, const float* bias, void* ctx, int B, int S, int C, int heads, int hdp,
                                          float eps, float scale, void* stream) {
  return fsvit_vit_ln_qkv_attention_dt(x, wqkv, kw, bias, ctx, B, S, C, heads, hdp, eps, scale, FSVIT_BF16, stream);
}
extern "C" int fsvit_vit_ln_qkv_attention_dt(const void* x, const void* wqkv, int kw, const float* bias, void* ctx, int B, int S, int C, int heads, int hdp,
                                          float eps, float scale, int dtype, void* stream) {
  const int kdt = dtype;
  if (!half_dtype(dtype)) return fail(FSVIT_ERR_ARG, "fsvit_vit_ln_qkv_attention: 16-bit storage only (bf16 / f16)");
  if (!x || !wqkv || !ctx) return fail(FSVIT_ERR_ARG, "null argument");
  if (!K(vit_attn_rows_supported)(1, C, heads, hdp, S) || kw < C)
    return fail(FSVIT_ERR_ARG, "fsvit_vit_ln_qkv_attention: built for C = 384, head dim 64, S <= 256");
  hipStream_t st = (hipStream_t)stream;
  void* img = nullptr;
  HIP_TRY(hipMalloc(&img, K(ln_gemm_rows_image_bytes)(C, 3 * heads * hdp)));
  int rc = K(launch_qkv_attn_rows_pack)(wqkv, kw, img, C, heads, hdp, st);
  if (rc == 0) rc = K(launch_vit_attn_rows)(x, ctx, img, bias, B, S, C, heads, hdp, eps, scale, st);
  (void)hipStreamSynchronize(st);
  (void)hipFree(img);
  if (rc != 0) return hipfail((hipError_t)rc, "fsvit_vit_ln_qkv_attention");
  return 0;
}

extern "C" int fsvit_op_attention_route(int S, int hdp, int dtype) {
  const int kdt = dtype;
  if (!known_dtype(dtype)) return -1;
  return K(attention_route)(S, hdp, kg(dtype));
}

extern "C" int fsvit_attention(const void* qkv, void* ctx, int B, int S, int heads, int hdp, float scale, int dtype, void* stream) {
  const int kdt = dtype;
  if (!known_dtype(dtype)) return fail(FSVIT_ERR_ARG, "unknown dtype %d", dtype);
  if (!qkv || !ctx) return fail(FSVIT_ERR_ARG, "null argument");
  if (B < 0 || heads < 1) return fail(FSVIT_ERR_ARG, "fsvit_attention: B = %d, heads = %d (B >= 0, heads >= 1)", B, heads);
  if (K(attention_route)(S, hdp, kg(dtype)) < 0)
    return fail(FSVIT_ERR_ARG, "fsvit_attention: no kernel covers S = %d, hdp = %d in dtype %d (fsvit.h)", S, hdp, dtype);
  int rc = K(launch_attention)(qkv, ctx, B, S, heads, hdp, scale, kg(dtype), (hipStream_t)stream);
  if (rc != 0) return hipfail((hipError_t)rc, "attention");
  return 0;
}

extern "C" int fsvit_im2col27(const float* x, void* out, int B, int H, int W, int dtype, void* stream) {
  const int kdt = dtype;
  if (!known_dtype(dtype)) return fail(FSVIT_ERR_ARG, "unknown dtype %d", dtype);
  if (!x || !out || (H & 1) || (W & 1)) return fail(FSVIT_ERR_ARG, "bad argument");
  RC_TRY(K(launch_im2col27)(x, out, B, H, W, H / 2, W / 2, kd(dtype), (hipStream_t)stream));
  return 0;
}

extern "C" int fsvit_stem_conv1(const float* x, const void* w, int kw, const float* bias, void* patches, void* c1, int B, int H, int W, void* stream) {
  return fsvit_stem_conv1_dt(x, w, kw, bias, patches, c1, B, H, W, FSVIT_BF16, stream);
}
extern "C" int fsvit_stem_conv1_dt(const float* x, const void* w, int kw, const float* bias, void* patches, void* c1, int B, int H, int W, int dtype, void* stream) {
  const int kdt = dtype;
  if (!half_dtype(dtype)) return fail(FSVIT_ERR_ARG, "fsvit_stem_conv1: 16-bit storage only (bf16 / f16)");
  if (!x || !w || !patches || !c1 || kw < 32) return fail(FSVIT_ERR_ARG, "bad argument");
  if (H != W || !K(stem_conv1_supported)(1, H, 64)) return fail(FSVIT_ERR_ARG, "fsvit_stem_conv1: only 80x80 images, 64 output channels are built");
  RC_TRY(K(launch_stem_conv1)(x, patches, c1, w, kw, bias, B, (hipStream_t)stream, 0));
  return 0;
}

extern "C" int fsvit_maxpool2_pos(const void* in, const float* pos, void* out, int B, int OH, int OW, int C, int dtype, void* stream) {
  const int kdt = dtype;
  if (!known_dtype(dtype)) return fail(FSVIT_ERR_ARG, "unknown dtype %d", dtype);
  if (!in || !out || C % 4) return fail(FSVIT_ERR_ARG, "bad argument");
  RC_TRY(K(launch_maxpool2_pos)(in, pos, out, B, OH, OW, C, kd(dtype), (hipStream_t)stream));
  return 0;
}

extern "C" int fsvit_pool_affine(const void* x, const float* scale, const float* shift, float* feat, int B, int HW, int C,
                                 int dtype, void* stream) {
  const int kdt = dtype;
  if (!known_dtype(dtype)) return fail(FSVIT_ERR_ARG, "unknown dtype %d", dtype);
  if (!x || !scale || !shift || !feat || C % 4 || C < 4 || HW < 1)
    return fail(FSVIT_ERR_ARG, "fsvit_pool_affine: null argument, C %% 4 != 0 or HW < 1 (the mean over no positions divides by zero)");
  RC_TRY(K(launch_pool_affine)(x, scale, shift, feat, B, HW, C, kd(dtype), (hipStream_t)stream));
  return 0;
}

extern "C" const char* fsvit_kernel_name(int kernel_id, int dtype) {
#define FSVIT_KERNEL_NAMES(T)                                                                                                                              \
  {"gemm256_kernel", "conv_gemm_v2_kernel<" T ",128,64,2,2,3>", "conv_gemm_v2_kernel<" T ",128,32,4,1,3>", "im2col27_kernel<" T ">", "maxpool2_pos_kernel<" T ">", \
   "attention_v2_kernel<" T ",...>", "pool_affine_kernel<" T ">", "proto_head_kernel", "stage1_block_kernel", "conv_gemm_v2_kernel<" T ",128,128,2,2,2>",          \
   "patchify_kernel<" T ">", "layernorm_kernel<" T ">", "conv3x3_halo_kernel", "mlp_rows_kernel", "-", "qkv_attn_kernel", "stem_conv1_kernel",                   \
   "stage1_ring_kernel", "ln_gemm_rows_kernel", "qkv_attn_rows_kernel", "vit_attn_rows_kernel"}
  static const char* const names[3][21] = {FSVIT_KERNEL_NAMES("float"), FSVIT_KERNEL_NAMES("__bf16"), FSVIT_KERNEL_NAMES("_Float16")};
#undef FSVIT_KERNEL_NAMES
  static const char* x2n[] = {"gemm256_x2_kernel", "conv_gemm_v2_kernel<f32x2l,128,64,2,2,3>", "conv_gemm_v2_kernel<f32x2l,128,32,4,1,3>", "", "", "", "", "", "", "conv_gemm_v2_kernel<f32x2l,128,128,2,2,2>"};
  if (kernel_id < 0 || kernel_id > 20) return "?";
  if (kernel_id == KID_STAGE1RING && kd(dtype) == 1) return "stage1_w4_kernel";
  if (is_x2(dtype)) return kernel_id == 14 ? "gconv3x3_x2_kernel" : (kernel_id == 0 || kernel_id == 1 || kernel_id == 2 || kernel_id == 9) ? x2n[kernel_id] : names[0][kernel_id];
  return names[dtype == FSVIT_F32 ? 0 : dtype == FSVIT_F16 ? 2 : 1][kernel_id];
}

extern "C" int fsvit_encoder_profile_begin(void* hv) {
  EngineBase* h = static_cast<EngineBase*>(hv);
  if (!h) return fail(FSVIT_ERR_ARG, "null argument");
  h->prof.clear();
  h->prof_last = nullptr;
  h->profiling = true;
  return 0;
}

extern "C" int fsvit_encoder_profile_end(void* hv, fsvit_prof_rec* out, int max_recs, int* n_out) {
  EngineBase* h = static_cast<EngineBase*>(hv);
  if (!h || !out || !n_out) return fail(FSVIT_ERR_ARG, "null argument");
  h->profiling = false;
  std::vector<fsvit_prof_rec> agg;
  hipEvent_t freed = nullptr;
  for (ProfEntry& e : h->prof) {
    HIP_TRY(hipEventSynchronize(e.e1));
    float ms = 0.f;
    HIP_TRY(hipEventElapsedTime(&ms, e.e0, e.e1));
    size_t k = 0;
    for (; k < agg.size(); ++k)
      if (e.layer == agg[k].layer && e.kernel == agg[k].kernel_id) break;
    if (k == agg.size()) {
      fsvit_prof_rec r;
      memset(&r, 0, sizeof(r));
      snprintf(r.layer, sizeof(r.layer), "%s", e.layer.c_str());
      r.kernel_id = e.kernel;
      agg.push_back(r);
    }
    agg[k].flops += e.flops;
    agg[k].ms += ms;
    agg[k].launches += 1;
  }
  for (ProfEntry& e : h->prof) {
    if (e.e0 != freed) (void)hipEventDestroy(e.e0);
    (void)hipEventDestroy(e.e1);
    freed = e.e1;
  }
  h->prof.clear();
  h->prof_last = nullptr;
  *n_out = (int)agg.size();
  if ((int)agg.size() > max_recs) return fail(FSVIT_ERR_ARG, "profile has %zu records, buffer holds %d", agg.size(), max_recs);
  for (size_t i = 0; i < agg.size(); ++i) out[i] = agg[i];
  return 0;
}

struct VitBlock {
  Layer qkv, proj, fc1, fc2;
  void* mlp_img = nullptr;
  float* mlp_b1 = nullptr;
  void* qkv_img = nullptr;
  void* attn_img = nullptr;
};

struct fsvit_vit : EngineBase {
  fsvit_vit_cfg cfg;
  int D = 0, S = 0, np = 0, npw = 0, Kp = 0, hd = 0, hdp = 0, hid = 0;
  Layer pe;
  float *pos_patch = nullptr;
  float *cls_pos0 = nullptr;
  float *ng = nullptr, *nb = nullptr;
  std::vector<VitBlock> blocks;
};

namespace {

std::vector<double> add_vec(const std::vector<double>& a, const float* b, int n) {
  std::vector<double> r(n);
  for (int i = 0; i < n; ++i) r[i] = a[i] + (double)b[i];
  return r;
}

int pack_vit_blocks(EngineBase* h, const SD& sd, int depth, int D, int heads, int hd, int hdp, int hid, int S, bool qkv_bias, double res_scale,
                    std::vector<VitBlock>* blocks_out) {
  std::vector<VitBlock>& blocks = *blocks_out;
  std::vector<int> rowmap(3 * heads * hd), colmap(heads * hd);
  for (int x = 0; x < 3; ++x)
    for (int y = 0; y < heads; ++y)
// ... 370 lines not shown
```

few-shot-vit_amd/csrc/kernels_decl.inc:

```
namespace FSVIT_DECL_NS {
using namespace fsvit_types;


int launch_im2col27(const float* x_nchw, void* out, int B, int H, int W, int OH, int OW, int dtype, hipStream_t s);
bool stem_conv1_supported(int dtype, int img, int C0);
int launch_stem_conv1(const float* x_nchw, void* patches, void* c1, const void* w, int kw, const float* bias, int B, hipStream_t s, int c1_planar = 0);
int launch_maxpool2_pos(const void* in, const float* pos, void* out, int B, int OH, int OW, int C, int dtype, hipStream_t s);

int launch_attention(const void* qkv, void* ctx, int B, int S, int heads, int hdp, float scale, int dtype, hipStream_t s);
int attention_route(int S, int hdp, int dtype);
size_t attention_lds_bytes(int S, int hdp, int dtype);
int attention_padded_head_dim(int hd, int S, int dtype);

int launch_pool_affine(const void* x, const float* scale, const float* shift, float* feat, int B, int HW, int C, int dtype, hipStream_t s);

bool stage1_ring_supported(int dtype, int C1, int hid, int group, int H1);
int launch_stage1_ring(const void* x, void* y, const void* w1, const float* b1, const void* w2, const void* w3, int B, int H, int W, hipStream_t s, const void* w3s = nullptr);
int launch_stage1_ring16(const void* x, void* y, const void* w1, const float* b1, const void* w2, const void* w3, int B, int H, int W, hipStream_t s);
int launch_stage1_w4(const void* x, void* y, const void* w1, const float* b1, const void* w2, const void* w3, int B, int H, int W, hipStream_t s, const void* w3s = nullptr);
int launch_stage1_w4_prescale(const void* w, void* ws, int n, hipStream_t s);
int launch_stage1_ring_block_train(const void* x, void* out, const void* w1f, const float* b1f, const void* w2, const void* w3, void* h1, void* g1, void* h2, void* g2,
                                   void* xn, const float* sa, const float* sb, const float* scale, float* stats, int B, int H, int W, hipStream_t s);
int launch_stage1_ring_dgrad(const void* dz3, void* dxn, const void* w3t, const void* w2t, const void* w1t, const void* g2, const void* g1, void* dz2, void* dz1,
                             int B, int H, int W, hipStream_t s);

bool mlp_rows_supported(int dtype, int C, int hid);
bool mlp_rows_proj_supported(int C, int hid, int KC);
size_t mlp_rows_image_bytes(int C, int hid, int KC);
int launch_mlp_pack(const void* w1, int k1w, const float* b1, const void* w2, int k2w, const void* wp, int kpw, int KC, void* wimg, float* b1img, int C,
                    int hid, hipStream_t s);
int launch_mlp_rows(const void* x, void* y, const void* wimg, const float* b1img, const float* b2, const void* ctx, int KC, int M, int C, int hid,
                    hipStream_t s);
bool mlp_rows_ln_supported(int dtype, int C, int hid, int KC);
int launch_mlp_rows_ln(const void* x, void* y, const void* wimg, const float* b1img, const float* bproj, const float* b2, const void* ctx, int KC, int M,
                       int C, int hid, float eps, hipStream_t s);

bool ln_gemm_rows_supported(int dtype, int C, int N);
size_t ln_gemm_rows_image_bytes(int C, int N);
int launch_ln_gemm_pack(const void* w, int kw, void* wimg, int C, int N, hipStream_t s);
int launch_ln_gemm_rows(const void* x, void* y, const void* wimg, const float* bias, int M, int C, int N, float eps, hipStream_t s);
bool gemm_rows_supported(int dtype, int C, int N);
int launch_gemm_rows(const void* x, void* y, const void* wimg, const float* bias, int M, int C, int N, hipStream_t s);

bool patch_embed_rows_supported(int dtype, int Ci, int H, int N);
int launch_patch_embed_rows(const void* x, void* y, const void* wimg, const float* bias, const float* pos, int B, int H, int Ci, int N, hipStream_t s);

bool qkv_attn_rows_supported(int dtype, int C, int heads, int hdp, int S);
int launch_qkv_attn_rows_pack(const void* w, int kw, void* wimg, int C, int heads, int hdp, hipStream_t s);
int launch_qkv_attn_rows(const void* x, void* ctx, const void* wimg, const float* bias, int B, int S, int C, int heads, int hdp, float scale, hipStream_t s);
bool vit_attn_rows_supported(int dtype, int C, int heads, int hdp, int S);
int launch_vit_attn_rows(const void* x, void* ctx, const void* wimg, const float* bias, int B, int S, int C, int heads, int hdp, float eps, float scale, hipStream_t s);

bool qkv_attn_supported(int dtype, int C, int heads, int hdp, int S);
size_t qkv_attn_image_bytes();
int launch_qkv_attn_pack(const void* w, int kw, void* img, hipStream_t s);
int launch_qkv_attn(const void* x, void* ctx, const void* wimg, const float* bias, int B, int S, float scale, hipStream_t s);

int launch_tokens_to_f32(const void* in, const float* scale, const float* shift, float* out, size_t n, int C, int dtype, hipStream_t s);
int launch_add_f32_into(void* inout, const float* add, size_t n, int dtype, hipStream_t s);

int launch_patchify(const float* x_nchw, void* out, int B, int img, int p, int Kp, int dtype, hipStream_t s);
int launch_cls_pos(const float* cls_plus_pos0, void* tokens, int B, int S, int D, int dtype, hipStream_t s);
int launch_layernorm(const void* x, void* y, int M, int D, float eps, int dtype, hipStream_t s);
int launch_final_ln_cls(const void* tokens, const float* gamma, const float* beta, float* feat, int B, int S, int D, float eps, int dtype, hipStream_t s);
int launch_final_ln_map(const void* tokens, const float* gamma, const float* beta, float* feat, float* map, int B, int S, int D, float eps, int dtype, hipStream_t s);

bool wgrad3x3_supported(int dtype, int O, int Ig, int groups, int W);
size_t wgrad3x3_scratch_bytes(int O, int Ig, int groups, int M, int dtype = 1);
bool wgrad1x1_supported(int dtype, int N, int C);
int wgrad1x1_splits(int N, int C, int M, int dtype = 1);
int launch_wgrad1x1(const void* x, int xld, int C, const void* dz, int zld, int N, float* y, int M, int Kc_pad, hipStream_t s, int dtype = 1);
bool gconv3x3_supported(int dtype, int O, int Ig, int groups, int KH, int KW, int stride, int pad, int W);
int launch_gconv3x3(const void* x, const void* w_packed, int Kw, void* y, int B, int H, int W, hipStream_t s, void* y2 = nullptr, const void* mul = nullptr);
int launch_wgrad3x3(const void* x, int xld, const void* dz, int zld, float* dw, float* scratch, int B, int H, int W, int O, int Ig, int groups, hipStream_t s,
                    int* defer = nullptr, int dtype = 1);

}
```

few-shot-vit_amd/csrc/stem.hip:

```cpp
#include "fsvit_common.h"
#include "kernels.h"

namespace FSVIT_NS {

template <typename T>
__global__ __launch_bounds__(256) void im2col27_kernel(const float* __restrict__ x, T* __restrict__ out,
                                                       int B, int H, int W, int OH, int OW) {
  const int m = blockIdx.x * 256 + threadIdx.x;
  const int M = B * OH * OW;
  if (m >= M) return;
  const int b = m / (OH * OW);
  const int rem = m - b * OH * OW;
  const int oy = rem / OW, ox = rem - oy * OW;
  const float* xb = x + (size_t)b * 3 * H * W;
  float v[32];
#pragma unroll
  for (int ky = 0; ky < 3; ++ky) {
    const int iy = oy * 2 - 1 + ky;
#pragma unroll
    for (int kx = 0; kx < 3; ++kx) {
      const int ix = ox * 2 - 1 + kx;
      const bool ok = (unsigned)iy < (unsigned)H && (unsigned)ix < (unsigned)W;
#pragma unroll
      for (int c = 0; c < 3; ++c)
        v[(ky * 3 + kx) * 3 + c] = ok ? xb[(size_t)c * H * W + (size_t)iy * W + ix] : 0.0f;
    }
  }
#pragma unroll
  for (int k = 27; k < 32; ++k) v[k] = 0.0f;
  T* o = out + (size_t)m * 32;
#pragma unroll
  for (int k = 0; k < 32; k += 4) store4<T>(o + k, f32x4{v[k], v[k + 1], v[k + 2], v[k + 3]});
}

template <typename T>
__global__ __launch_bounds__(256) void maxpool2_pos_kernel(const T* __restrict__ in, const float* __restrict__ pos,
                                                           T* __restrict__ out, int B, int OH, int OW, int C) {
  const int c4 = C / 4;
  const size_t total = (size_t)B * OH * OW * c4;
  for (size_t idx = (size_t)blockIdx.x * 256 + threadIdx.x; idx < total; idx += (size_t)gridDim.x * 256) {
    const int cq = (int)(idx % c4);
    const size_t pix = idx / c4;
    const int ox = (int)(pix % OW);
    const size_t t2 = pix / OW;
    const int oy = (int)(t2 % OH);
    const size_t b = t2 / OH;
    const int W = OW * 2;
    const T* p00 = in + ((b * OH * 2 + oy * 2) * W + ox * 2) * C + cq * 4;
    f32x4 a = load4<T>(p00), b1 = load4<T>(p00 + C), c1 = load4<T>(p00 + (size_t)W * C), d = load4<T>(p00 + (size_t)W * C + C);
    f32x4 v;
#pragma unroll
    for (int e = 0; e < 4; ++e) v[e] = fmaxf(fmaxf(a[e], b1[e]), fmaxf(c1[e], d[e]));
    if (pos) v += *reinterpret_cast<const f32x4*>(pos + (size_t)(oy * OW + ox) * C + cq * 4);
    store4<T>(out + pix * C + cq * 4, v);
  }
}

namespace stem1 {
constexpr int IMG = 80, OH = 40, ROWS = 8;
constexpr int IR = 2 * ROWS + 1, LPAD = 4, ICP = IMG + 2 * LPAD;
constexpr int PLANE = IR * ICP;
constexpr int NW = 4;
}

__global__ __launch_bounds__(stem1::NW * 64) void stem_conv1_kernel(const float* __restrict__ x, bf16* __restrict__ patches, bf16* __restrict__ c1,
                                                                    const bf16* __restrict__ w, const int kw, const float* __restrict__ bias, const int c1_planar) {
  using namespace stem1;
  __shared__ __attribute__((aligned(16))) bf16 tile[3 * PLANE];
  const int t = threadIdx.x, lane = t & 63, wave = t >> 6;
  const int m = lane & 15, lq = lane >> 4;
  const int b = blockIdx.x / (OH / ROWS), strip = blockIdx.x % (OH / ROWS);
  const int oy0 = strip * ROWS, iy0 = 2 * oy0 - 1;
  const float* xb = x + (size_t)b * 3 * IMG * IMG;

  for (int i = t; i < 3 * IR * (IMG / 4); i += NW * 64) {
    const int c = i / (IR * (IMG / 4)), r = (i / (IMG / 4)) % IR, q4 = i % (IMG / 4);
    const int iy = iy0 + r;
    f32x4 v = {0.f, 0.f, 0.f, 0.f};
    if (iy >= 0 && iy < IMG) v = *reinterpret_cast<const f32x4*>(xb + ((size_t)c * IMG + iy) * IMG + q4 * 4);
    *reinterpret_cast<bf16x4*>(tile + c * PLANE + r * ICP + LPAD + q4 * 4) = bf16x4{(bf16)v[0], (bf16)v[1], (bf16)v[2], (bf16)v[3]};
  }
  for (int i = t; i < 3 * IR; i += NW * 64)
    *reinterpret_cast<bf16x4*>(tile + (i / IR) * PLANE + (i % IR) * ICP) = bf16x4{(bf16)0.0f, (bf16)0.0f, (bf16)0.0f, (bf16)0.0f};
  u32x4 wf[4];
  f32x4 bv[4];
#pragma unroll
  for (int ct = 0; ct < 4; ++ct) {
    const int p = ct >> 1, hh = ct & 1;
    wf[ct] = *reinterpret_cast<const u32x4*>(w + (size_t)(32 * p + 8 * (m >> 2) + 4 * hh + (m & 3)) * kw + 8 * lq);
    bv[ct] = bias ? *reinterpret_cast<const f32x4*>(bias + 32 * p + 8 * lq + 4 * hh) : f32x4{0.f, 0.f, 0.f, 0.f};
  }
  int koff[8];
#pragma unroll
  for (int j = 0; j < 8; ++j) {
    const int k = 8 * lq + j, tap = k / 3, c = k - 3 * tap;
    koff[j] = k < 27 ? c * PLANE + (tap / 3) * ICP + (tap % 3) : -1;
  }
  __syncthreads();

  const size_t prow0 = ((size_t)b * OH + oy0) * OH;
  for (int tl = wave; tl < ROWS * OH / 16; tl += NW) {
    const int pix = tl * 16 + m, oy = pix / OH, ox = pix - oy * OH;
    const int org = (2 * oy) * ICP + 2 * ox + LPAD - 1;
    unsigned short e[8];
#pragma unroll
    for (int j = 0; j < 8; ++j) e[j] = koff[j] >= 0 ? __builtin_bit_cast(unsigned short, tile[org + koff[j]]) : (unsigned short)0;
    const u32x4 pf = {(unsigned)e[0] | ((unsigned)e[1] << 16), (unsigned)e[2] | ((unsigned)e[3] << 16), (unsigned)e[4] | ((unsigned)e[5] << 16),
                      (unsigned)e[6] | ((unsigned)e[7] << 16)};
    *reinterpret_cast<u32x4*>(patches + (prow0 + pix) * 32 + 8 * lq) = pf;
#pragma unroll
    for (int p = 0; p < 2; ++p) {
      const f32x4 a0 = mma_chunk<bf16>(wf[2 * p], pf, bv[2 * p]), a1 = mma_chunk<bf16>(wf[2 * p + 1], pf, bv[2 * p + 1]);
      bf16x8 o;
#pragma unroll
      for (int q = 0; q < 4; ++q) {
        o[q] = (bf16)fmaxf(a0[q], 0.1f * a0[q]);
        o[4 + q] = (bf16)fmaxf(a1[q], 0.1f * a1[q]);
      }
      if (c1_planar) *reinterpret_cast<bf16x8*>(c1 + ((((size_t)b * OH + oy0 + oy) * 8 + 4 * p + lq) * OH + ox) * 8) = o;
      else *reinterpret_cast<bf16x8*>(c1 + (prow0 + pix) * 64 + 32 * p + 8 * lq) = o;
    }
  }
}

bool stem_conv1_supported(int dtype, int img, int C0) { return dtype == 1 && img == stem1::IMG && C0 == 64; }

int launch_stem_conv1(const float* x, void* patches, void* c1, const void* w, int kw, const float* bias, int B, hipStream_t s, int c1_planar) {
  if (B <= 0) return 0;
  hipLaunchKernelGGL(stem_conv1_kernel, dim3(B * (stem1::OH / stem1::ROWS)), dim3(stem1::NW * 64), 0, s, x, (bf16*)patches, (bf16*)c1, (const bf16*)w, kw, bias, c1_planar);
  return (int)hipGetLastError();
}

int launch_im2col27(const float* x, void* out, int B, int H, int W, int OH, int OW, int dtype, hipStream_t s) {
  const int M = B * OH * OW;
  if (M <= 0) return 0;
  return with_elem(dtype, [&](auto e) { return launch(im2col27_kernel<elem_t<decltype(e)>>, (M + 255) / 256, 256, 0, s, x, out, B, H, W, OH, OW); });
}

int launch_maxpool2_pos(const void* in, const float* pos, void* out, int B, int OH, int OW, int C, int dtype, hipStream_t s) {
  const size_t total = (size_t)B * OH * OW * (C / 4);
  if (total == 0) return 0;
  size_t nb = (total + 255) / 256;
  if (nb > 8192) nb = 8192;
  return with_elem(dtype, [&](auto e) { return launch(maxpool2_pos_kernel<elem_t<decltype(e)>>, (unsigned)nb, 256, 0, s, in, pos, out, B, OH, OW, C); });
}

}
```

few-shot-vit_amd/engine.py:

```python
import ctypes as C
import os
import sys
from typing import Dict, Optional

import numpy as np
import torch

from . import _lib

DTYPES = {'f32': _lib.F32, 'parity': _lib.F32, 'fp32': _lib.F32, 'bf16': _lib.BF16, 'f16': _lib.F16, 'fp16': _lib.F16,
          'bf16x2': _lib.BF16X2, 'f16x2': _lib.F16X2}
TORCH_DTYPE = {_lib.F32: torch.float32, _lib.BF16: torch.bfloat16, _lib.F16: torch.float16, _lib.BF16X2: torch.float32, _lib.F16X2: torch.float32}
EVAL_ONLY = (_lib.F16, _lib.F16X2)


_tensor_generation = {}


def bump_weight_generation(tensors) -> None:
    for t in tensors:
        if t is not None:
            p = t.data_ptr()
            _tensor_generation[p] = _tensor_generation.get(p, 0) + 1

# ... 624 lines not shown
        _require_cuda(x, ctx, wp, bp, w1, b1, w2, b2)
        dt = ops._dt16(x, ctx, wp, w1, w2)
        lib = _lib.load()
        y = ops._out(out, x, x.shape[1])
        with torch.cuda.device(x.device):
            _lib.check(lib.fsvit_vit_block_tail_dt(_ptr(x), _ptr(y), _ptr(ctx), _ptr(wp), wp.shape[-1], ctx.shape[1], _ptr(bp), _ptr(w1), w1.shape[-1],
                                                   _ptr(b1), _ptr(w2), w2.shape[-1], _ptr(b2), x.shape[0], x.shape[1], w1.shape[0], float(eps),
                                                   dt, _stream_ptr(x.device)))
        return y

    @staticmethod
    def mlp_rows(x, w1, b1, w2, b2=None, out=None):
        _require_cuda(x, w1, w2)
        dt = ops._dt16(x, w1, w2)
        lib = _lib.load()
        y = ops._out(out, x, x.shape[1])
        with torch.cuda.device(x.device):
            _lib.check(lib.fsvit_mlp_rows_dt(_ptr(x), _ptr(y), _ptr(w1), w1.shape[-1], _ptr(b1), _ptr(w2), w2.shape[-1], _ptr(b2),
                                             x.shape[0], x.shape[1], w1.shape[0], dt, _stream_ptr(x.device)))
        return y

    @staticmethod
    def attention(qkv, B, S, heads, hdp, scale, numerics=None, out=None):
        _require_cuda(qkv)
        if numerics is not None:
            if numerics not in ('bf16x2', 'f16x2'):
                raise ValueError(f"numerics: None, 'bf16x2' or 'f16x2', got {numerics!r}")
            if qkv.dtype != torch.float32:
                raise TypeError(f'the two-limb modes read fp32 rows, got {qkv.dtype}')
        if tuple(qkv.shape) != (B * S, 3 * heads * hdp) or not qkv.is_contiguous():
            raise ValueError(f'qkv must be a contiguous [{B * S}, {3 * heads * hdp}] tensor')
        lib = _lib.load()
        ctx = ops._out(out, qkv, heads * hdp)
        with torch.cuda.device(qkv.device):
            _lib.check(lib.fsvit_attention(_ptr(qkv), _ptr(ctx), B, S, heads, hdp, float(scale), DTYPES[numerics] if numerics else ops._dt(qkv),
                                           _stream_ptr(qkv.device)))
        return ctx

    @staticmethod
    def qkv_attention(x, wqkv, bias, B, S, heads, hdp, scale):
        _require_cuda(x, wqkv)
        dt = ops._dt16(x, wqkv)
        lib = _lib.load()
        ctx = torch.empty(B * S, heads * hdp, dtype=x.dtype, device=x.device)
        with torch.cuda.device(x.device):
            _lib.check(lib.fsvit_qkv_attention_dt(_ptr(x), _ptr(wqkv), wqkv.shape[-1], _ptr(bias), _ptr(ctx), B, S, x.shape[1], heads, hdp,
                                                  float(scale), dt, _stream_ptr(x.device)))
        return ctx

    @staticmethod
    def vit_ln_qkv_attention(x, wqkv, bias, B, S, heads, hdp, scale, eps=1e-6):
        _require_cuda(x, wqkv)
        dt = ops._dt16(x, wqkv)
        ctx = torch.empty(B * S, heads * hdp, dtype=x.dtype, device=x.device)
        with torch.cuda.device(x.device):
            _lib.check(_lib.load().fsvit_vit_ln_qkv_attention_dt(_ptr(x), _ptr(wqkv), wqkv.shape[-1], _ptr(bias), _ptr(ctx), B, S, x.shape[1], heads, hdp,
                                                                 float(eps), float(scale), dt, _stream_ptr(x.device)))
        return ctx

    @staticmethod
    def im2col27(x, dtype):
        _require_cuda(x)
        lib = _lib.load()
        B, _, H, W = x.shape
        out = torch.empty(B * (H // 2) * (W // 2), 32, dtype=dtype, device=x.device)
        with torch.cuda.device(x.device):
            _lib.check(lib.fsvit_im2col27(_ptr(x.contiguous()), _ptr(out), B, H, W, ops._dt(out), _stream_ptr(x.device)))
        return out

    @staticmethod
    def stem_conv1(x, w, bias):
        _require_cuda(x, w)
        if x.dtype != torch.float32:
            raise TypeError(f'stem_conv1 reads the fp32 image, got {x.dtype}')
        dt = ops._dt16(w)
        lib = _lib.load()
        B, _, H, W = x.shape
        patches = torch.empty(B * (H // 2) * (W // 2), 32, dtype=w.dtype, device=x.device)
        c1 = torch.empty(B * (H // 2) * (W // 2), 64, dtype=w.dtype, device=x.device)
        with torch.cuda.device(x.device):
            _lib.check(lib.fsvit_stem_conv1_dt(_ptr(x.contiguous()), _ptr(w), w.shape[-1], _ptr(bias), _ptr(patches), _ptr(c1), B, H, W, dt,
                                               _stream_ptr(x.device)))
        return patches, c1

    @staticmethod
    def maxpool2_pos(x, pos):
        _require_cuda(x)
        lib = _lib.load()
        B, H, W, Cc = x.shape
        out = torch.empty(B, H // 2, W // 2, Cc, dtype=x.dtype, device=x.device)
        with torch.cuda.device(x.device):
            _lib.check(lib.fsvit_maxpool2_pos(_ptr(x), _ptr(pos), _ptr(out), B, H // 2, W // 2, Cc, ops._dt(x), _stream_ptr(x.device)))
        return out

    @staticmethod
    def pool_affine(x, scale, shift):
        _require_cuda(x)
        lib = _lib.load()
        B, HW, Cc = x.shape
        out = torch.empty(B, Cc, dtype=torch.float32, device=x.device)
        with torch.cuda.device(x.device):
            _lib.check(lib.fsvit_pool_affine(_ptr(x), _ptr(scale), _ptr(shift), _ptr(out), B, HW, Cc, ops._dt(x), _stream_ptr(x.device)))
        return out

    @staticmethod
    def attention_backward(qkv, dctx, B, S, heads, hd, hdp, scale, out=None):
        _require_cuda(qkv, dctx)
        if qkv.dtype not in (torch.float32, torch.bfloat16):
            raise TypeError(f'attention_backward is built for torch.float32 and torch.bfloat16, got {qkv.dtype}')
        if dctx.dtype != qkv.dtype:
            raise TypeError(f'qkv is {qkv.dtype} but dctx is {dctx.dtype}')
        if tuple(qkv.shape) != (B * S, 3 * heads * hdp) or tuple(dctx.shape) != (B * S, heads * hdp) or not qkv.is_contiguous() or not dctx.is_contiguous():
            raise ValueError(f'qkv / dctx must be contiguous [{B * S}, {3 * heads * hdp}] / [{B * S}, {heads * hdp}] tensors')
        lib = _lib.load()
        dqkv = ops._out(out, qkv, 3 * heads * hdp)
        with torch.cuda.device(qkv.device):
            _lib.check(lib.fsvit_attention_backward(_ptr(qkv), _ptr(dctx), _ptr(dqkv), B, S, heads, hd, hdp, float(scale),
                                                    ops._dt(qkv), _stream_ptr(qkv.device)))
        return dqkv

    @staticmethod
    def _head_in(*ts):
        return tuple(t.detach().contiguous().float() for t in ts)

    @staticmethod
    def proto_head_backward(feat_shot, feat_query, dlogits, temp, method='cos'):
        if method not in ('cos', 'sqr'):
            raise ValueError(method)
        _require_cuda(feat_shot, feat_query, dlogits)
        lib = _lib.load()
        feat_shot, feat_query, dlogits = ops._head_in(feat_shot, feat_query, dlogits)
        E, way, shot, D = feat_shot.shape
        Q = feat_query.shape[1]
        dev = feat_shot.device
        ds, dq = torch.empty_like(feat_shot), torch.empty_like(feat_query)
        dt = torch.empty(E, dtype=torch.float32, device=dev)
        with torch.cuda.device(dev):
            if isinstance(temp, torch.Tensor) and temp.is_cuda:
                _lib.check(lib.fsvit_proto_head_backward_devtemp(_ptr(feat_shot), _ptr(feat_query), _ptr(dlogits), E, way, shot, Q, D,
                                                                 _ptr(ops._head_in(temp)[0]), _lib.HEAD_COS if method == 'cos' else _lib.HEAD_SQR,
                                                                 _ptr(ds), _ptr(dq), _ptr(dt), _stream_ptr(dev)))
            else:
                fn = lib.fsvit_proto_head_backward if method == 'cos' else lib.fsvit_proto_head_backward_sqr
                _lib.check(fn(_ptr(feat_shot), _ptr(feat_query), _ptr(dlogits), E, way, shot, Q, D, float(temp), _ptr(ds), _ptr(dq), _ptr(dt),
                              _stream_ptr(dev)))
        return ds, dq, dt.sum()

    @staticmethod
    def conv1x1_wgrad(x, dz, limbs='bf16'):
        _require_cuda(x, dz)
        lib = _lib.load()
        assert x.dtype == dz.dtype and x.dtype in (torch.bfloat16, torch.float16, torch.float32) and x.shape[0] == dz.shape[0]
        x, dz = x.contiguous(), dz.contiguous()
        dw = torch.empty(dz.shape[1], x.shape[1], dtype=torch.float32, device=x.device)
        dt = {torch.bfloat16: _lib.BF16, torch.float16: _lib.F16, torch.float32: _lib.BF16X2 if limbs == 'bf16' else _lib.F16X2}[x.dtype]
        with torch.cuda.device(x.device):
            _lib.check(lib.fsvit_conv1x1_wgrad(_ptr(x), _ptr(dz), _ptr(dw), x.shape[0], dz.shape[1], x.shape[1], dt, _stream_ptr(x.device)))
        return dw

    @staticmethod
    def conv3x3_wgrad(x_nhwc, dz, O, Ig, groups, limbs='bf16'):
        _require_cuda(x_nhwc, dz)
        lib = _lib.load()
        assert x_nhwc.dtype == dz.dtype and x_nhwc.dtype in (torch.bfloat16, torch.float16, torch.float32)
        B, H, W, C = x_nhwc.shape
        assert C == groups * Ig and dz.shape == (B, H, W, O)
# ... 616 lines not shown
```

include/fsvit.h:

```cpp
#ifndef FSVIT_H
#define FSVIT_H
#include <stddef.h>
#include <stdint.h>

#ifdef __cplusplus
extern "C" {
#endif

enum { FSVIT_F32 = 0, FSVIT_BF16 = 1, FSVIT_F16 = 2, FSVIT_BF16X2 = 3, FSVIT_F16X2 = 4 };
enum { FSVIT_ACT_NONE = 0, FSVIT_ACT_GELU = 1, FSVIT_ACT_LRELU = 2,
       FSVIT_ACT_MUL = 3  };
enum { FSVIT_HEAD_COS = 0, FSVIT_HEAD_SQR = 1, FSVIT_HEAD_DOT = 2 };
enum {
  FSVIT_ERR_ARG = -1,
  FSVIT_ERR_KEY = -2,
  FSVIT_ERR_IMG_SIZE = -3,
  FSVIT_ERR_WORKSPACE = -4
};

const char* fsvit_last_error(void);
const char* fsvit_version(void);

typedef struct fsvit_visformer fsvit_visformer;

typedef struct fsvit_tensor {
  const char* name;
  const float* data;
  int ndim;
  int64_t shape[4];
} fsvit_tensor;

typedef struct fsvit_visformer_cfg {
  int img_size;
  int init_channels;
  int embed_dim;
  int depth[3];
  int num_heads;
  float mlp_ratio;
  int group;
  float bn_eps;
} fsvit_visformer_cfg;

int fsvit_visformer_create(const fsvit_visformer_cfg* cfg, const fsvit_tensor* state_dict, int n_tensors,
                           int dtype, fsvit_visformer** out);
void fsvit_visformer_destroy(fsvit_visformer* h);
int fsvit_visformer_out_dim(const fsvit_visformer* h);
int fsvit_visformer_dtype(const fsvit_visformer* h);
size_t fsvit_visformer_workspace_bytes(const fsvit_visformer* h, int chunk_images);
int fsvit_visformer_forward(fsvit_visformer* h, const float* x_nchw_dev, int n_img, int img_h, int img_w,
                            float* feat_dev, void* ws_dev, size_t ws_bytes, void* stream);
int fsvit_encoder_set_tap(void* encoder, const char* name, void* dst_dev, size_t bytes);

typedef struct fsvit_prof_rec {
  char layer[48];
  int kernel_id;
  int launches;
  double flops;
  double ms;
} fsvit_prof_rec;
int fsvit_encoder_profile_begin(void* encoder);
int fsvit_encoder_profile_end(void* encoder, fsvit_prof_rec* out, int max_recs, int* n_out);
const char* fsvit_kernel_name(int kernel_id, int dtype);

typedef struct fsvit_vit fsvit_vit;
typedef struct fsvit_vit_cfg {
  int img_size;
  int patch_size;
  int embed_dim;
  int depth;
  int num_heads;
  float mlp_ratio;
  float ln_eps;
} fsvit_vit_cfg;
int fsvit_vit_create(const fsvit_vit_cfg* cfg, const fsvit_tensor* state_dict, int n_tensors, int dtype, fsvit_vit** out);
void fsvit_vit_destroy(fsvit_vit* h);
int fsvit_vit_out_dim(const fsvit_vit* h);
size_t fsvit_vit_workspace_bytes(const fsvit_vit* h, int chunk_images);
int fsvit_vit_forward(fsvit_vit* h, const float* x_nchw_dev, int n_img, int img_h, int img_w, float* feat_dev,
                      void* ws_dev, size_t ws_bytes, void* stream);

typedef struct fsvit_lvvit fsvit_lvvit;
typedef struct fsvit_lvvit_cfg {
  int img_size;
  int stem_channels;
  int embed_dim;
  int depth;
  int num_heads;
  float mlp_ratio;
  float skip_lam;
  float ln_eps;
  float bn_eps;
} fsvit_lvvit_cfg;
int fsvit_lvvit_create(const fsvit_lvvit_cfg* cfg, const fsvit_tensor* state_dict, int n_tensors, int dtype, fsvit_lvvit** out);
void fsvit_lvvit_destroy(fsvit_lvvit* h);
int fsvit_lvvit_out_dim(const fsvit_lvvit* h);
size_t fsvit_lvvit_workspace_bytes(const fsvit_lvvit* h, int chunk_images);
int fsvit_lvvit_forward(fsvit_lvvit* h, const float* x_nchw_dev, int n_img, int img_h, int img_w, float* feat_dev,
                        void* ws_dev, size_t ws_bytes, void* stream);
int fsvit_lvvit_forward_map(fsvit_lvvit* h, const float* x_nchw_dev, int n_img, int img_h, int img_w, float* feat_dev, float* tokens_dev, void* ws_dev,
                            size_t ws_bytes, void* stream);

int fsvit_stem96_conv(const void* x_dev, const void* w_dev, const float* bias_dev, const void* x2_dev, int x2_cstride, int K2, void* y_dev,
                      int B, int H, int W, int pool, int dtype, void* stream);

int fsvit_proto_head(const float* feat_shot_dev, const float* feat_query_dev, int E, int way, int shot, int Q, int D,
                     float temp, int method, float* logits_dev, float* acc_dev, float* loss_dev, void* stream);

int fsvit_proto_head_devtemp(const float* feat_shot_dev, const float* feat_query_dev, int E, int way, int shot, int Q, int D,
                             const float* temp_dev, int method, float* logits_dev, float* acc_dev, float* loss_dev, void* stream);

int fsvit_meta_baseline_forward(void* encoder , const float* x_shot_dev, const float* x_query_dev,
                                int E, int way, int shot, int Q, int img_h, int img_w, float temp, int method,
                                float* logits_dev, float* acc_dev, float* loss_dev, float* feat_dev,
                                void* ws_dev, size_t ws_bytes, void* stream);

int fsvit_conv_gemm(const void* x_dev, const void* w_dev, const float* bias_dev, const void* res_dev,
                    const float* pos_dev, void* y_dev, int B, int H, int W, int Cin, int x_cstride,
                    int KH, int KW, int stride, int pad, int N, int y_cstride, int Kw, int groups,
                    int act, int res_first, int dtype, void* stream);
int fsvit_conv_stem_tail(const void* x_dev, const void* w_dev, const float* bias_dev, const float* pos_dev, const void* x2_dev, int x2_cstride,
                         int K2, void* y_dev, int B, int H, int W, int Cin, int N, int Kw, int dtype, void* stream);
int fsvit_attention(const void* qkv_dev, void* ctx_dev, int B, int S, int heads, int hdp, float scale,
                    int dtype, void* stream);
int fsvit_op_attention_route(int S, int hdp, int dtype);
int fsvit_qkv_attention(const void* x_dev, const void* wqkv_dev, int kw, const float* bias_dev, void* ctx_dev, int B, int S, int C,
                        int heads, int hdp, float scale, void* stream);
int fsvit_vit_ln_qkv_attention(const void* x_dev, const void* wqkv_dev, int kw, const float* bias_dev, void* ctx_dev, int B, int S, int C,
                               int heads, int hdp, float eps, float scale, void* stream);
int fsvit_stage1_block(const void* x_dev, void* y_dev, const void* w1_dev, const float* b1_dev, const void* w2_dev,
                       const void* w3_dev, int B, void* stream);
int fsvit_stage1_block_hw(const void* x_dev, void* y_dev, const void* w1_dev, const float* b1_dev, const void* w2_dev, const void* w3_dev, int B, int H, int W,
                          int dtype, void* stream);
int fsvit_mlp_rows(const void* x_dev, void* y_dev, const void* w1_dev, int k1w, const float* b1_dev, const void* w2_dev, int k2w,
                   const float* b2_dev, int M, int C, int hid, void* stream);
int fsvit_proj_mlp_rows(const void* x_dev, void* y_dev, const void* ctx_dev, const void* wp_dev, int kpw, int KC, const void* w1_dev, int k1w,
                        const float* b1_dev, const void* w2_dev, int k2w, const float* b2_dev, int M, int C, int hid, void* stream);
int fsvit_vit_block_tail(const void* x_dev, void* y_dev, const void* ctx_dev, const void* wp_dev, int kpw, int KC, const float* bp_dev,
                         const void* w1_dev, int k1w, const float* b1_dev, const void* w2_dev, int k2w, const float* b2_dev, int M, int C, int hid,
                         float eps, void* stream);
int fsvit_ln_linear_rows(const void* x_dev, void* y_dev, const void* w_dev, int kw, const float* b_dev, int M, int C, int N, float eps, void* stream);
int fsvit_patch_embed2x2(const void* x_dev, void* y_dev, const void* w_dev, int kw, const float* bias_dev, const float* pos_dev, int B, int H, int Ci,
                         int N, void* stream);
int fsvit_mlp_rows_dt(const void* x_dev, void* y_dev, const void* w1_dev, int k1w, const float* b1_dev, const void* w2_dev, int k2w,
                      const float* b2_dev, int M, int C, int hid, int dtype, void* stream);
int fsvit_proj_mlp_rows_dt(const void* x_dev, void* y_dev, const void* ctx_dev, const void* wp_dev, int kpw, int KC, const void* w1_dev, int k1w,
                           const float* b1_dev, const void* w2_dev, int k2w, const float* b2_dev, int M, int C, int hid, int dtype, void* stream);
int fsvit_vit_block_tail_dt(const void* x_dev, void* y_dev, const void* ctx_dev, const void* wp_dev, int kpw, int KC, const float* bp_dev,
                            const void* w1_dev, int k1w, const float* b1_dev, const void* w2_dev, int k2w, const float* b2_dev, int M, int C, int hid,
                            float eps, int dtype, void* stream);
int fsvit_ln_linear_rows_dt(const void* x_dev, void* y_dev, const void* w_dev, int kw, const float* b_dev, int M, int C, int N, float eps, int dtype,
                            void* stream);
int fsvit_patch_embed2x2_dt(const void* x_dev, void* y_dev, const void* w_dev, int kw, const float* bias_dev, const float* pos_dev, int B, int H, int Ci,
                            int N, int dtype, void* stream);
int fsvit_qkv_attention_dt(const void* x_dev, const void* wqkv_dev, int kw, const float* bias_dev, void* ctx_dev, int B, int S, int C,
                           int heads, int hdp, float scale, int dtype, void* stream);
int fsvit_vit_ln_qkv_attention_dt(const void* x_dev, const void* wqkv_dev, int kw, const float* bias_dev, void* ctx_dev, int B, int S, int C,
                                  int heads, int hdp, float eps, float scale, int dtype, void* stream);
int fsvit_stem_conv1_dt(const float* x_nchw_dev, const void* w_dev, int kw, const float* bias_dev, void* patches_dev, void* c1_dev,
                        int B, int H, int W, int dtype, void* stream);
int fsvit_visformer_last_tokens(fsvit_visformer* h, const void* ws_dev, size_t ws_bytes, int n_img, float* tokens_dev, void* stream);
int fsvit_linear_forward(const float* x_dev, const float* w_dev, const float* b_dev, float* y_dev, int M, int N, int K, void* stream);
int fsvit_linear_backward(const float* dy_dev, const float* x_dev, const float* w_dev, float* dx_dev, int accumulate_dx, float* dw_dev,
                          float* db_dev, int M, int N, int K, void* stream);
int fsvit_token_softlabel(const float* teacher_logits_dev, float* soft_dev, int B, int T, int C, int k, int bp, double smoothing, void* stream);
int fsvit_soft_target_ce(const float* logits_dev, const float* target_dev, float* row_loss_dev, float* dlogits_dev, int R, int C,
                         float grad_scale, void* stream);
int fsvit_row_normalize(const float* x_dev, float* y_dev, float* inv_norm_dev, int R, int D, void* stream);
int fsvit_row_normalize_backward(const float* y_dev, const float* inv_norm_dev, const float* dy_dev, float* dx_dev, int R, int D, void* stream);
int fsvit_adamw_step(float* p_dev, const float* g_dev, float* m_dev, float* v_dev, size_t n, float lr, float beta1, float beta2, float eps,
                     float weight_decay, int step, void* stream);
int fsvit_adamw_step_multi(const void* items_dev, int n_items, size_t max_numel, float lr, float beta1, float beta2, float eps, float weight_decay, int step,
                           void* stream);

int fsvit_im2col27(const float* x_nchw_dev, void* out_dev, int B, int H, int W, int dtype, void* stream);
int fsvit_stem_conv1(const float* x_nchw_dev, const void* w_dev, int kw, const float* bias_dev, void* patches_dev, void* c1_dev,
                     int B, int H, int W, void* stream);
int fsvit_maxpool2_pos(const void* in_dev, const float* pos_dev, void* out_dev, int B, int OH, int OW, int C,
                       int dtype, void* stream);
int fsvit_pool_affine(const void* x_dev, const float* scale_dev, const float* shift_dev, float* feat_dev,
                      int B, int HW, int C, int dtype, void* stream);

typedef struct fsvit_param {
  const char* name;
  float* data;
  float* grad;
  int64_t numel;
} fsvit_param;
typedef struct fsvit_visformer_trainer fsvit_visformer_trainer;
int fsvit_visformer_train_tokens(fsvit_visformer_trainer* t, float* tokens_dev, void* stream);
int fsvit_visformer_train_set_token_grad(fsvit_visformer_trainer* t, const float* dtokens_dev);
int fsvit_visformer_trainer_create(const fsvit_visformer_cfg* cfg, int dtype, fsvit_visformer_trainer** out);
void fsvit_visformer_trainer_destroy(fsvit_visformer_trainer* t);
size_t fsvit_visformer_trainer_workspace_bytes(fsvit_visformer_trainer* t, const fsvit_param* params, int n_params, int n_img,
                                               float drop_path_rate);
int fsvit_visformer_trainer_set_freeze_bn(fsvit_visformer_trainer* t, int on);

int fsvit_visformer_train_forward(fsvit_visformer_trainer* t, const fsvit_param* params, int n_params, const float* x_nchw_dev,
                                  int n_img, int img_h, int img_w, float drop_path_rate, const float* masks_dev, float* feat_dev,
                                  void* ws_dev, size_t ws_bytes, void* stream);
int fsvit_visformer_train_backward(fsvit_visformer_trainer* t, const fsvit_param* params, int n_params, const float* dfeat_dev,
                                   void* stream);
typedef struct fsvit_vit_trainer fsvit_vit_trainer;
int fsvit_vit_trainer_create(const fsvit_vit_cfg* cfg, int dtype, fsvit_vit_trainer** out);
void fsvit_vit_trainer_destroy(fsvit_vit_trainer* t);
int fsvit_vit_trainer_droppath_calls(const fsvit_vit_trainer* t, float drop_path_rate);
size_t fsvit_vit_trainer_workspace_bytes(fsvit_vit_trainer* t, const fsvit_param* params, int n_params, int n_img, float drop_path_rate);
int fsvit_vit_train_forward(fsvit_vit_trainer* t, const fsvit_param* params, int n_params, const float* x_nchw_dev, int n_img, int img_h, int img_w,
                            float drop_path_rate, const float* masks_dev, float* feat_dev, void* ws_dev, size_t ws_bytes, void* stream);
int fsvit_vit_train_backward(fsvit_vit_trainer* t, const fsvit_param* params, int n_params, const float* dfeat_dev, void* stream);

typedef struct fsvit_lvvit_trainer fsvit_lvvit_trainer;
int fsvit_lvvit_trainer_create(const fsvit_lvvit_cfg* cfg, int dtype, fsvit_lvvit_trainer** out);
void fsvit_lvvit_trainer_destroy(fsvit_lvvit_trainer* t);
int fsvit_lvvit_trainer_droppath_calls(const fsvit_lvvit_trainer* t, float drop_path_rate);
size_t fsvit_lvvit_trainer_workspace_bytes(fsvit_lvvit_trainer* t, const fsvit_param* params, int n_params, int n_img, float drop_path_rate);
int fsvit_lvvit_trainer_set_freeze_bn(fsvit_lvvit_trainer* t, int on);
int fsvit_lvvit_train_forward(fsvit_lvvit_trainer* t, const fsvit_param* params, int n_params, const float* x_nchw_dev, int n_img, int img_h, int img_w,
                              float drop_path_rate, const float* masks_dev, float* feat_dev, void* ws_dev, size_t ws_bytes, void* stream);
int fsvit_lvvit_train_backward(fsvit_lvvit_trainer* t, const fsvit_param* params, int n_params, const float* dfeat_dev, void* stream);
int fsvit_lvvit_train_tokens(fsvit_lvvit_trainer* t, float* tokens_dev, void* stream);
int fsvit_lvvit_train_set_token_grad(fsvit_lvvit_trainer* t, const float* dtokens_dev);

int fsvit_proto_head_backward(const float* feat_shot_dev, const float* feat_query_dev, const float* dlogits_dev, int E, int way,
                              int shot, int Q, int D, float temp, float* dfeat_shot_dev, float* dfeat_query_dev,
                              float* dtemp_per_episode_dev, void* stream);
int fsvit_proto_head_backward_sqr(const float* feat_shot_dev, const float* feat_query_dev, const float* dlogits_dev, int E, int way,
                                  int shot, int Q, int D, float temp, float* dfeat_shot_dev, float* dfeat_query_dev,
                                  float* dtemp_per_episode_dev, void* stream);
int fsvit_proto_head_backward_devtemp(const float* feat_shot_dev, const float* feat_query_dev, const float* dlogits_dev, int E, int way,
                                      int shot, int Q, int D, const float* temp_dev, int method, float* dfeat_shot_dev,
                                      float* dfeat_query_dev, float* dtemp_per_episode_dev, void* stream);
int fsvit_proto_head_ce(const float* feat_shot_dev, const float* feat_query_dev, const long long* labels_dev, int E, int way, int shot, int Q, int D, float temp,
                        const float* temp_dev, int method, float* logits_dev, float* dlogits_dev, float* acc_per_episode_dev, float* loss_per_episode_dev,
                        float* loss_acc_mean_dev, unsigned* ticket_dev, void* stream);
int fsvit_proto_head_ce_backward(const float* feat_shot_dev, const float* feat_query_dev, const float* dlogits_dev, const float* dloss_dev, int E, int way,
                                 int shot, int Q, int D, float temp, const float* temp_dev, int method, float* dfeat_shot_dev, float* dfeat_query_dev,
                                 float* dtemp_dev, unsigned* ticket_dev, void* stream);
int fsvit_sgd_step_multi(const void* items_dev, int n_items, size_t max_numel, float lr, float momentum, float weight_decay, int first_step,
                         void* stream);

int fsvit_sgd_step(float* param_dev, const float* grad_dev, float* momentum_buf_dev, size_t n, float lr, float momentum,
                   float weight_decay, int first_step, void* stream);
// ... 112 lines not shown
```

Measured before the change: 4488 episodes/s.

## Fuse stem conv1, conv2 and conv3 into a persistent per-image pipeline kernel

Adds a persistent stem_pipe kernel. Each block processes whole images in turn: it runs the conv1 stem into a per-block scratch region, then the two 3x3 halo convolutions, with device-scope fence handoffs between stages. This replaces the separate sliced launches for most of the chunk. The intent is to keep the intermediate c1/c2 activations small and L2-resident and to remove launch and inter-kernel gaps. The cost is less parallelism within each image and a fixed grid of 256. The halo conv body is refactored into a device function so it can take a tile start and step, and the remaining images beyond a multiple of the grid still use the old path.

```diff
diff --git a/few-shot-vit_amd/_lib.py b/few-shot-vit_amd/_lib.py
--- a/few-shot-vit_amd/_lib.py
+++ b/few-shot-vit_amd/_lib.py
@@ -50,6 +50,7 @@
     'fsvit_visformer_out_dim': (_i, [_vp]),
     'fsvit_visformer_dtype': (_i, [_vp]),
     'fsvit_visformer_workspace_bytes': (_sz, [_vp, _i]),
+    'fsvit_visformer_plan_bytes': (_sz, [C.POINTER(VisformerCfg), _i, _i]),
     'fsvit_visformer_forward': (_i, [_vp, _fp, _i, _i, _i, _fp, _vp, _sz, _vp]),
     'fsvit_vit_create': (_i, [C.POINTER(VitCfg), C.POINTER(Tensor), _i, _i, C.POINTER(_vp)]),
     'fsvit_vit_destroy': (None, [_vp]),
@@ -105,6 +106,9 @@
     'fsvit_im2col27': (_i, [_fp, _vp, _i, _i, _i, _i, _vp]),
     'fsvit_stem_conv1': (_i, [_fp, _vp, _i, _fp, _vp, _vp, _i, _i, _i, _vp]),
     'fsvit_stem_conv1_dt': (_i, [_fp, _vp, _i, _fp, _vp, _vp, _i, _i, _i, _i, _vp]),
+    'fsvit_stem_pipe_scratch_bytes': (_sz, []),
+    'fsvit_stem_pipe_grid': (_i, []),
+    'fsvit_stem_pipe': (_i, [_fp, _fp, _i, _i, _vp, _i, _fp, _vp, _i, _fp, _vp, _i, _fp, _fp, _vp, _vp, _i, _i, _vp]),
     'fsvit_maxpool2_pos': (_i, [_vp, _fp, _vp, _i, _i, _i, _i, _i, _vp]),
     'fsvit_pool_affine': (_i, [_vp, _fp, _fp, _fp, _i, _i, _i, _i, _vp]),
     'fsvit_visformer_trainer_create': (_i, [C.POINTER(VisformerCfg), _i, C.POINTER(_vp)]),
diff --git a/few-shot-vit_amd/csrc/conv3x3_halo.hip b/few-shot-vit_amd/csrc/conv3x3_halo.hip
--- a/few-shot-vit_amd/csrc/conv3x3_halo.hip
+++ b/few-shot-vit_amd/csrc/conv3x3_halo.hip
@@ -7,7 +7,7 @@
 
 namespace FSVIT_NS {
 
-__device__ __attribute__((aligned(256))) unsigned char g_zero_page_halo[256];
+static __device__ __attribute__((aligned(256))) unsigned char g_zero_page_halo[256];
 #define HWAIT(vm) asm volatile("s_waitcnt vmcnt(" #vm ") lgkmcnt(0)" ::: "memory")
 
 template <int CTRL>
@@ -27,14 +27,14 @@
 static_assert(LDS_BYTES == 160 * 1024, "the two halo buffers and the weight ring fill the LDS exactly");
 }
 
-template <int CIN, bool FUSE_TAIL, bool STATS = false, int CREAL = CIN>
-__global__ __launch_bounds__(512, 2) void conv3x3_halo_kernel(const ConvGemmParams p, const int n_tiles) {
+template <int CIN, bool FUSE_TAIL, bool STATS = false, int CREAL = CIN, typename TileStep>
+__device__ __forceinline__ void conv3x3_halo_tiles(const ConvGemmParams& p, const int n_tiles, const int tile0, const TileStep tile_step, const int t) {
   using namespace halo;
   extern __shared__ __attribute__((aligned(16))) unsigned char smem[];
   constexpr int NH = CIN / 64;
   constexpr int NKM = 9 * NH, NKT = NKM + (FUSE_TAIL ? 1 : 0);
   constexpr int MT = 5, NT = 4;
-  const int t = threadIdx.x, lane = t & 63;
+  const int lane = t & 63;
   const int wave = __builtin_amdgcn_readfirstlane(t >> 6);
   const int wm = wave >> 1, wn = wave & 1;
   const int lrow = lane & 15, lq = lane >> 4;
@@ -93,9 +93,9 @@
 #pragma unroll
     for (int j = 0; j < NT; ++j) acc[i][j] = f32x4{0.f, 0.f, 0.f, 0.f};
 
-  int tix = blockIdx.x;
+  int tix = tile0;
   if (tix >= n_tiles) return;
-  const int my_tiles = (n_tiles - tix + (int)gridDim.x - 1) / (int)gridDim.x;
+  const int my_tiles = (n_tiles - tix + tile_step() - 1) / tile_step();
   int steps_left = my_tiles * NKT;
 
   auto wk_of = [&](int q) { return q >= NKM ? NKM : (NH == 2 ? (q >= 9 ? (q - 9) * 2 + 1 : q * 2) : q); };
@@ -122,7 +122,7 @@
   };
 
   while (true) {
-    const int tnext = tix + (int)gridDim.x;
+    const int tnext = tix + tile_step();
     const bool has_next = tnext < n_tiles;
     const int b = tix / tiles_per_img, r0 = (tix - b * tiles_per_img) * TR;
     u32x4 xf0[MT], wf0[NT];
@@ -387,6 +387,13 @@
     }
   }
 }
+
+template <int CIN, bool FUSE_TAIL, bool STATS = false, int CREAL = CIN>
+__global__ __launch_bounds__(512, 2) void conv3x3_halo_kernel(const ConvGemmParams p, const int n_tiles) {
+  conv3x3_halo_tiles<CIN, FUSE_TAIL, STATS, CREAL>(p, n_tiles, (int)blockIdx.x, []() { return (int)gridDim.x; }, (int)threadIdx.x);
+}
+
+#ifndef FSVIT_HALO_DEVICE_ONLY
 
 bool conv3x3_halo_eligible(const ConvGemmParams& p, int dtype) {
   if (dtype != 1) return false;
@@ -432,5 +439,6 @@
   if (p.stats) return p.Cin == 64 ? launch_halo_t<64, false, true>(p, stream) : launch_halo_t<128, false, true>(p, stream);
   return p.Cin == 64 ? launch_halo_t<64, false>(p, stream) : launch_halo_t<128, false>(p, stream);
 }
-
-}
+#endif
+
+}
diff --git a/few-shot-vit_amd/csrc/engine.hip b/few-shot-vit_amd/csrc/engine.hip
--- a/few-shot-vit_amd/csrc/engine.hip
+++ b/few-shot-vit_amd/csrc/engine.hip
@@ -332,10 +332,9 @@
   return 0;
 }
 
-int build(fsvit_visformer* h, const SD& sd) {
+int visformer_geometry(fsvit_visformer* h) {
   const int kdt = h->dtype;
   const fsvit_visformer_cfg& cf = h->cfg;
-  const double eps = cf.bn_eps;
   const int epc = 16 / h->es;
   const int D = cf.embed_dim;
   h->C0 = cf.init_channels; h->C1 = D / 2; h->C2 = D; h->C3 = h->out_dim = D * 2;
@@ -355,6 +354,15 @@
   if (!is_pow2(h->C0) || !is_pow2(h->C1) || !is_pow2(h->C2) || !is_pow2(Cg))
     return fail(FSVIT_ERR_ARG, "multi-tap conv input channels must be powers of two");
   if (h->H2 * h->H2 > 128) return fail(FSVIT_ERR_ARG, "attention supports at most 128 tokens (img_size <= 88)");
+  return 0;
+}
+
+int build(fsvit_visformer* h, const SD& sd) {
+  const int kdt = h->dtype;
+  const fsvit_visformer_cfg& cf = h->cfg;
+  const double eps = cf.bn_eps;
+  RC_TRY(visformer_geometry(h));
+  const int epc = 16 / h->es, Cg = h->hid1 / cf.group;
 
   std::vector<double> nob;
   WRound wr;
@@ -584,6 +592,8 @@
 
 struct Plan {
   size_t patches, c1, c2;
+  size_t pipe;
+  int pipe_images;
   size_t ha, hb;
   size_t qkv, ctx, hid;
   size_t x1, x1b, x2, x3;
@@ -591,6 +601,12 @@
 };
 
 size_t align256(size_t v) { return (v + 255) / 256 * 256; }
+
+int stem_pipe_images(const fsvit_visformer* h, size_t Bc) {
+  const int kdt = h->dtype, G = K(stem_pipe_grid)();
+  if (!K(stem_pipe_supported)(kd(kdt), h->cfg.img_size, h->C0, h->C1) || Bc < (size_t)4 * G) return 0;
+  return (int)(Bc / G) * G;
+}
 
 Plan make_plan(const fsvit_visformer* h, size_t Bc) {
   Plan p;
@@ -606,6 +622,11 @@
   p.patches = take(Bc * P0 * 32 * es);
   p.c1 = take(Bc * P0 * h->C0 * es);
   p.c2 = take(Bc * P0 * h->C1 * es);
+  p.pipe_images = stem_pipe_images(h, Bc);
+  {
+    const int kdt = h->dtype;
+    p.pipe = take(p.pipe_images ? (size_t)K(stem_pipe_grid)() * K(stem_pipe_scratch_bytes)() : 0);
+  }
   size_t hi = off;
   off = scratch0;
   p.ha = take(Bc * P1 * h->hid1 * es);
@@ -647,7 +668,7 @@
   return 0;
 }
 
-enum { KID_GEMM256 = 0, KID_GEMM64 = 1, KID_GEMM32 = 2, KID_IM2COL = 3, KID_MAXPOOL = 4, KID_ATTN = 5, KID_POOL = 6, KID_HEAD = 7, KID_STAGE1 = 8, KID_GEMM128 = 9, KID_HALO = 12, KID_MLPROWS = 13, KID_QKVATTN = 15, KID_STEMCONV1 = 16, KID_GCONV_X2 = 14, KID_STAGE1RING = 17, KID_LNGEMM = 18, KID_QKVATTNROWS = 19, KID_VITATTNROWS = 20 };
+enum { KID_GEMM256 = 0, KID_GEMM64 = 1, KID_GEMM32 = 2, KID_IM2COL = 3, KID_MAXPOOL = 4, KID_ATTN = 5, KID_POOL = 6, KID_HEAD = 7, KID_STAGE1 = 8, KID_GEMM128 = 9, KID_HALO = 12, KID_MLPROWS = 13, KID_QKVATTN = 15, KID_STEMCONV1 = 16, KID_GCONV_X2 = 14, KID_STAGE1RING = 17, KID_LNGEMM = 18, KID_QKVATTNROWS = 19, KID_VITATTNROWS = 20, KID_STEMPIPE = 21 };
 
 
 template <typename F>
@@ -694,12 +715,21 @@
   p3.x2 = patches; p3.x2_cstride = 32; p3.K2 = 32; p3.pool2 = 1;
   const bool planar = conv1_fused && K(conv_gemm_route)(p2, kg(kdt)) == 0 && K(conv_gemm_route)(p3, kg(kdt)) == 0;
   p2.x_planar = p2.y_planar = p3.x_planar = planar ? 1 : 0;
+  const bool planar_pipe = planar && K(stem_pipe_supported)(dt, img, h->C0, h->C1);
   if (planar) {
     const int S = stem_slice_images();
     const size_t s_pat = (size_t)h->H0 * h->H0 * 32 * es, s_c1 = (size_t)h->H0 * h->H0 * h->C0 * es, s_c2 = (size_t)h->H0 * h->H0 * h->C1 * es,
                  s_x1 = (size_t)h->H1 * h->H1 * h->C1 * es;
     const double fl1 = 2.0 * 27.0 * h->C0 * h->H0 * h->H0;
-    for (int g0 = 0; g0 < Bc; g0 += S) {
+    const int n_pipe = planar_pipe ? pl.pipe_images : 0;
+    if (n_pipe) {
+      ConvGemmParams q2 = p2, q3 = p3;
+      q2.B = q3.B = 1; q2.M = q2.OH * q2.OW; q3.M = q3.OH * q3.OW;
+      const double fl = fl1 + 2.0 * h->H0 * h->H0 * h->C1 * (9.0 * h->C0 + 9.0 * h->C1 + 27.0);
+      RC_TRY(timed(h, st, "stem.pipe", KID_STEMPIPE, fl * n_pipe, [&]() {
+        return K(launch_stem_pipe)(x, xsrc2, B1 < n_pipe ? B1 : n_pipe, n_pipe, h->conv1.w, h->conv1.Kw, h->conv1.bias, q2, q3, ws + pl.pipe, K(stem_pipe_grid)(), st); }));
+    }
+    for (int g0 = n_pipe; g0 < Bc; g0 += S) {
       const int g1 = g0 + S < Bc ? g0 + S : Bc;
       for (int part = 0; part < 2; ++part) {
         const int a = part == 0 ? g0 : (g0 > B1 ? g0 : B1), b = part == 0 ? (g1 < B1 ? g1 : B1) : g1;
@@ -883,6 +913,13 @@
 extern "C" int fsvit_visformer_out_dim(const fsvit_visformer* h) { return h ? h->out_dim : 0; }
 extern "C" int fsvit_visformer_dtype(const fsvit_visformer* h) { return h ? h->dtype : -1; }
 extern "C" size_t fsvit_visformer_workspace_bytes(const fsvit_visformer* h, int chunk_images) { return encoder_workspace_bytes(h, chunk_images); }
+extern "C" size_t fsvit_visformer_plan_bytes(const fsvit_visformer_cfg* cfg, int dtype, int chunk_images) {
+  if (!cfg || !known_dtype(dtype) || chunk_images <= 0 || cfg->num_heads < 1 || cfg->embed_dim < 2 || cfg->init_channels < 1) return 0;
+  fsvit_visformer h;
+  h.cfg = *cfg; h.img_size = cfg->img_size; h.dtype = dtype; h.es = storage_bytes(dtype);
+  if (visformer_geometry(&h) != 0) return 0;
+  return make_plan(&h, (size_t)chunk_images).total;
+}
 
 extern "C" int fsvit_encoder_set_tap(void* hv, const char* name, void* dst_dev, size_t bytes) {
   EngineBase* h = static_cast<EngineBase*>(hv);
@@ -1283,6 +1320,26 @@
   return 0;
 }
 
+extern "C" size_t fsvit_stem_pipe_scratch_bytes(void) { return fsvit::stem_pipe_scratch_bytes(); }
+extern "C" int fsvit_stem_pipe_grid(void) { return fsvit::stem_pipe_grid(); }
+extern "C" int fsvit_stem_pipe(const float* x, const float* xsrc2, int B1, int B, const void* w1, int kw1, const float* b1, const void* w2, int kw2, const float* b2,
+                               const void* w3, int kw3, const float* b3, const float* pos, void* scratch, void* x1, int grid, int dtype, void* stream) {
+  const int kdt = dtype;
+  if (!half_dtype(dtype)) return fail(FSVIT_ERR_ARG, "fsvit_stem_pipe: 16-bit storage only (bf16 / f16)");
+  if (!x || !w1 || !w2 || !w3 || !pos || !scratch || !x1 || B <= 0 || B1 < 0 || B1 > B || (B1 < B && !xsrc2) || kw1 < 32 || kw2 != 9 * 64 || kw3 != 9 * 128 + 64 ||
+      ((uintptr_t)scratch & 255))
+    return fail(FSVIT_ERR_ARG, "fsvit_stem_pipe: bad argument");
+  Layer L2, L3;
+  L2.w = const_cast<void*>(w2); L2.bias = const_cast<float*>(b2); L2.N = 128; L2.K = 9 * 64; L2.Kw = kw2; L2.groups = 1;
+  L3.w = const_cast<void*>(w3); L3.bias = const_cast<float*>(b3); L3.N = 128; L3.K = 9 * 128; L3.Kw = kw3; L3.groups = 1;
+  ConvGemmParams p2 = conv_params(L2, scratch, scratch, 1, 40, 40, 64, 64, 3, 3, 1, 1, 128, ACT_LRELU, nullptr, 0, nullptr);
+  ConvGemmParams p3 = conv_params(L3, scratch, x1, 1, 40, 40, 128, 128, 3, 3, 1, 1, 128, ACT_LRELU, nullptr, 0, pos);
+  p3.x2 = scratch; p3.x2_cstride = 32; p3.K2 = 32; p3.pool2 = 1;
+  p2.x_planar = p2.y_planar = p3.x_planar = 1;
+  RC_TRY(K(launch_stem_pipe)(x, xsrc2, B1, B, w1, kw1, b1, p2, p3, scratch, grid > 0 ? grid : K(stem_pipe_grid)(), (hipStream_t)stream));
+  return 0;
+}
+
 extern "C" int fsvit_maxpool2_pos(const void* in, const float* pos, void* out, int B, int OH, int OW, int C, int dtype, void* stream) {
   const int kdt = dtype;
   if (!known_dtype(dtype)) return fail(FSVIT_ERR_ARG, "unknown dtype %d", dtype);
@@ -1306,11 +1363,11 @@
   {"gemm256_kernel", "conv_gemm_v2_kernel<" T ",128,64,2,2,3>", "conv_gemm_v2_kernel<" T ",128,32,4,1,3>", "im2col27_kernel<" T ">", "maxpool2_pos_kernel<" T ">", \
    "attention_v2_kernel<" T ",...>", "pool_affine_kernel<" T ">", "proto_head_kernel", "stage1_block_kernel", "conv_gemm_v2_kernel<" T ",128,128,2,2,2>",          \
    "patchify_kernel<" T ">", "layernorm_kernel<" T ">", "conv3x3_halo_kernel", "mlp_rows_kernel", "-", "qkv_attn_kernel", "stem_conv1_kernel",                   \
-   "stage1_ring_kernel", "ln_gemm_rows_kernel", "qkv_attn_rows_kernel", "vit_attn_rows_kernel"}
-  static const char* const names[3][21] = {FSVIT_KERNEL_NAMES("float"), FSVIT_KERNEL_NAMES("__bf16"), FSVIT_KERNEL_NAMES("_Float16")};
+   "stage1_ring_kernel", "ln_gemm_rows_kernel", "qkv_attn_rows_kernel", "vit_attn_rows_kernel", "stem_pipe_kernel"}
+  static const char* const names[3][22] = {FSVIT_KERNEL_NAMES("float"), FSVIT_KERNEL_NAMES("__bf16"), FSVIT_KERNEL_NAMES("_Float16")};
 #undef FSVIT_KERNEL_NAMES
   static const char* x2n[] = {"gemm256_x2_kernel", "conv_gemm_v2_kernel<f32x2l,128,64,2,2,3>", "conv_gemm_v2_kernel<f32x2l,128,32,4,1,3>", "", "", "", "", "", "", "conv_gemm_v2_kernel<f32x2l,128,128,2,2,2>"};
-  if (kernel_id < 0 || kernel_id > 20) return "?";
+  if (kernel_id < 0 || kernel_id > KID_STEMPIPE) return "?";
   if (kernel_id == KID_STAGE1RING && kd(dtype) == 1) return "stage1_w4_kernel";
   if (is_x2(dtype)) return kernel_id == 14 ? "gconv3x3_x2_kernel" : (kernel_id == 0 || kernel_id == 1 || kernel_id == 2 || kernel_id == 9) ? x2n[kernel_id] : names[0][kernel_id];
   return names[dtype == FSVIT_F32 ? 0 : dtype == FSVIT_F16 ? 2 : 1][kernel_id];
diff --git a/few-shot-vit_amd/csrc/kernels_decl.inc b/few-shot-vit_amd/csrc/kernels_decl.inc
--- a/few-shot-vit_amd/csrc/kernels_decl.inc
+++ b/few-shot-vit_amd/csrc/kernels_decl.inc
@@ -5,6 +5,11 @@
 int launch_im2col27(const float* x_nchw, void* out, int B, int H, int W, int OH, int OW, int dtype, hipStream_t s);
 bool stem_conv1_supported(int dtype, int img, int C0);
 int launch_stem_conv1(const float* x_nchw, void* patches, void* c1, const void* w, int kw, const float* bias, int B, hipStream_t s, int c1_planar = 0);
+bool stem_pipe_supported(int dtype, int img, int C0, int C1);
+size_t stem_pipe_scratch_bytes();
+int stem_pipe_grid();
+int launch_stem_pipe(const float* x, const float* x2, int B1, int B, const void* w1, int kw1, const float* b1, const ConvGemmParams& p2, const ConvGemmParams& p3,
+                     void* scratch, int grid, hipStream_t s);
 int launch_maxpool2_pos(const void* in, const float* pos, void* out, int B, int OH, int OW, int C, int dtype, hipStream_t s);
 
 int launch_attention(const void* qkv, void* ctx, int B, int S, int heads, int hdp, float scale, int dtype, hipStream_t s);
diff --git a/few-shot-vit_amd/csrc/stem.hip b/few-shot-vit_amd/csrc/stem.hip
--- a/few-shot-vit_amd/csrc/stem.hip
+++ b/few-shot-vit_amd/csrc/stem.hip
@@ -1,5 +1,6 @@
 #include "fsvit_common.h"
 #include "kernels.h"
+#include "stem_conv1.h"
 
 namespace FSVIT_NS {
 
@@ -56,71 +57,16 @@
   }
 }
 
-namespace stem1 {
-constexpr int IMG = 80, OH = 40, ROWS = 8;
-constexpr int IR = 2 * ROWS + 1, LPAD = 4, ICP = IMG + 2 * LPAD;
-constexpr int PLANE = IR * ICP;
-constexpr int NW = 4;
-}
-
 __global__ __launch_bounds__(stem1::NW * 64) void stem_conv1_kernel(const float* __restrict__ x, bf16* __restrict__ patches, bf16* __restrict__ c1,
                                                                     const bf16* __restrict__ w, const int kw, const float* __restrict__ bias, const int c1_planar) {
   using namespace stem1;
   __shared__ __attribute__((aligned(16))) bf16 tile[3 * PLANE];
   const int t = threadIdx.x, lane = t & 63, wave = t >> 6;
-  const int m = lane & 15, lq = lane >> 4;
   const int b = blockIdx.x / (OH / ROWS), strip = blockIdx.x % (OH / ROWS);
-  const int oy0 = strip * ROWS, iy0 = 2 * oy0 - 1;
-  const float* xb = x + (size_t)b * 3 * IMG * IMG;
-
-  for (int i = t; i < 3 * IR * (IMG / 4); i += NW * 64) {
-    const int c = i / (IR * (IMG / 4)), r = (i / (IMG / 4)) % IR, q4 = i % (IMG / 4);
-    const int iy = iy0 + r;
-    f32x4 v = {0.f, 0.f, 0.f, 0.f};
-    if (iy >= 0 && iy < IMG) v = *reinterpret_cast<const f32x4*>(xb + ((size_t)c * IMG + iy) * IMG + q4 * 4);
-    *reinterpret_cast<bf16x4*>(tile + c * PLANE + r * ICP + LPAD + q4 * 4) = bf16x4{(bf16)v[0], (bf16)v[1], (bf16)v[2], (bf16)v[3]};
-  }
-  for (int i = t; i < 3 * IR; i += NW * 64)
-    *reinterpret_cast<bf16x4*>(tile + (i / IR) * PLANE + (i % IR) * ICP) = bf16x4{(bf16)0.0f, (bf16)0.0f, (bf16)0.0f, (bf16)0.0f};
-  u32x4 wf[4];
-  f32x4 bv[4];
-#pragma unroll
-  for (int ct = 0; ct < 4; ++ct) {
-    const int p = ct >> 1, hh = ct & 1;
-    wf[ct] = *reinterpret_cast<const u32x4*>(w + (size_t)(32 * p + 8 * (m >> 2) + 4 * hh + (m & 3)) * kw + 8 * lq);
-    bv[ct] = bias ? *reinterpret_cast<const f32x4*>(bias + 32 * p + 8 * lq + 4 * hh) : f32x4{0.f, 0.f, 0.f, 0.f};
-  }
-  int koff[8];
-#pragma unroll
-  for (int j = 0; j < 8; ++j) {
-    const int k = 8 * lq + j, tap = k / 3, c = k - 3 * tap;
-    koff[j] = k < 27 ? c * PLANE + (tap / 3) * ICP + (tap % 3) : -1;
-  }
+  stem_conv1_stage(x + (size_t)b * 3 * IMG * IMG, tile, strip, t);
+  const StemConv1Weights cw = stem_conv1_weights(w, kw, bias, lane);
   __syncthreads();
-
-  const size_t prow0 = ((size_t)b * OH + oy0) * OH;
-  for (int tl = wave; tl < ROWS * OH / 16; tl += NW) {
-    const int pix = tl * 16 + m, oy = pix / OH, ox = pix - oy * OH;
-    const int org = (2 * oy) * ICP + 2 * ox + LPAD - 1;
-    unsigned short e[8];
-#pragma unroll
-    for (int j = 0; j < 8; ++j) e[j] = koff[j] >= 0 ? __builtin_bit_cast(unsigned short, tile[org + koff[j]]) : (unsigned short)0;
-    const u32x4 pf = {(unsigned)e[0] | ((unsigned)e[1] << 16), (unsigned)e[2] | ((unsigned)e[3] << 16), (unsigned)e[4] | ((unsigned)e[5] << 16),
-                      (unsigned)e[6] | ((unsigned)e[7] << 16)};
-    *reinterpret_cast<u32x4*>(patches + (prow0 + pix) * 32 + 8 * lq) = pf;
-#pragma unroll
-    for (int p = 0; p < 2; ++p) {
-      const f32x4 a0 = mma_chunk<bf16>(wf[2 * p], pf, bv[2 * p]), a1 = mma_chunk<bf16>(wf[2 * p + 1], pf, bv[2 * p + 1]);
-      bf16x8 o;
-#pragma unroll
-      for (int q = 0; q < 4; ++q) {
-        o[q] = (bf16)fmaxf(a0[q], 0.1f * a0[q]);
-        o[4 + q] = (bf16)fmaxf(a1[q], 0.1f * a1[q]);
-      }
-      if (c1_planar) *reinterpret_cast<bf16x8*>(c1 + ((((size_t)b * OH + oy0 + oy) * 8 + 4 * p + lq) * OH + ox) * 8) = o;
-      else *reinterpret_cast<bf16x8*>(c1 + (prow0 + pix) * 64 + 32 * p + 8 * lq) = o;
-    }
-  }
+  stem_conv1_tiles(tile, patches + (size_t)b * OH * OH * 32, c1 + (size_t)b * OH * OH * 64, cw, strip, wave, lane, c1_planar);
 }
 
 bool stem_conv1_supported(int dtype, int img, int C0) { return dtype == 1 && img == stem1::IMG && C0 == 64; }
diff --git a/few-shot-vit_amd/csrc/stem_conv1.h b/few-shot-vit_amd/csrc/stem_conv1.h
--- /dev/null
+++ b/few-shot-vit_amd/csrc/stem_conv1.h
@@ -0,0 +1,77 @@
+#pragma once
+#include "fsvit_common.h"
+
+namespace FSVIT_NS {
+
+namespace stem1 {
+constexpr int IMG = 80, OH = 40, ROWS = 8;
+constexpr int IR = 2 * ROWS + 1, LPAD = 4, ICP = IMG + 2 * LPAD;
+constexpr int PLANE = IR * ICP;
+constexpr int NW = 4;
+constexpr int TILE_BYTES = 3 * PLANE * 2;
+}
+
+__device__ __forceinline__ void stem_conv1_stage(const float* __restrict__ xb, bf16* tile, const int strip, const int tg) {
+  using namespace stem1;
+  const int iy0 = 2 * strip * ROWS - 1;
+  for (int i = tg; i < 3 * IR * (IMG / 4); i += NW * 64) {
+    const int c = i / (IR * (IMG / 4)), r = (i / (IMG / 4)) % IR, q4 = i % (IMG / 4);
+    const int iy = iy0 + r;
+    f32x4 v = {0.f, 0.f, 0.f, 0.f};
+    if (iy >= 0 && iy < IMG) v = *reinterpret_cast<const f32x4*>(xb + ((size_t)c * IMG + iy) * IMG + q4 * 4);
+    *reinterpret_cast<bf16x4*>(tile + c * PLANE + r * ICP + LPAD + q4 * 4) = bf16x4{(bf16)v[0], (bf16)v[1], (bf16)v[2], (bf16)v[3]};
+  }
+  for (int i = tg; i < 3 * IR; i += NW * 64)
+    *reinterpret_cast<bf16x4*>(tile + (i / IR) * PLANE + (i % IR) * ICP) = bf16x4{(bf16)0.0f, (bf16)0.0f, (bf16)0.0f, (bf16)0.0f};
+}
+
+struct StemConv1Weights { u32x4 wf[4]; f32x4 bv[4]; };
+__device__ __forceinline__ StemConv1Weights stem_conv1_weights(const bf16* __restrict__ w, const int kw, const float* __restrict__ bias, const int lane) {
+  const int m = lane & 15, lq = lane >> 4;
+  StemConv1Weights r;
+#pragma unroll
+  for (int ct = 0; ct < 4; ++ct) {
+    const int p = ct >> 1, hh = ct & 1;
+    r.wf[ct] = *reinterpret_cast<const u32x4*>(w + (size_t)(32 * p + 8 * (m >> 2) + 4 * hh + (m & 3)) * kw + 8 * lq);
+    r.bv[ct] = bias ? *reinterpret_cast<const f32x4*>(bias + 32 * p + 8 * lq + 4 * hh) : f32x4{0.f, 0.f, 0.f, 0.f};
+  }
+  return r;
+}
+
+__device__ __forceinline__ void stem_conv1_tiles(const bf16* tile, bf16* __restrict__ patches, bf16* __restrict__ c1, const StemConv1Weights& cw, const int strip,
+                                                 const int gw, const int lane, const int c1_planar) {
+  using namespace stem1;
+  const int m = lane & 15, lq = lane >> 4;
+  const int oy0 = strip * ROWS;
+  int koff[8];
+#pragma unroll
+  for (int j = 0; j < 8; ++j) {
+    const int k = 8 * lq + j, tap = k / 3, c = k - 3 * tap;
+    koff[j] = k < 27 ? c * PLANE + (tap / 3) * ICP + (tap % 3) : -1;
+  }
+  const size_t prow0 = (size_t)oy0 * OH;
+  for (int tl = gw; tl < ROWS * OH / 16; tl += NW) {
+    const int pix = tl * 16 + m, oy = pix / OH, ox = pix - oy * OH;
+    const int org = (2 * oy) * ICP + 2 * ox + LPAD - 1;
+    unsigned short e[8];
+#pragma unroll
+    for (int j = 0; j < 8; ++j) e[j] = koff[j] >= 0 ? __builtin_bit_cast(unsigned short, tile[org + koff[j]]) : (unsigned short)0;
+    const u32x4 pf = {(unsigned)e[0] | ((unsigned)e[1] << 16), (unsigned)e[2] | ((unsigned)e[3] << 16), (unsigned)e[4] | ((unsigned)e[5] << 16),
+                      (unsigned)e[6] | ((unsigned)e[7] << 16)};
+    *reinterpret_cast<u32x4*>(patches + (prow0 + pix) * 32 + 8 * lq) = pf;
+#pragma unroll
+    for (int p = 0; p < 2; ++p) {
+      const f32x4 a0 = mma_chunk<bf16>(cw.wf[2 * p], pf, cw.bv[2 * p]), a1 = mma_chunk<bf16>(cw.wf[2 * p + 1], pf, cw.bv[2 * p + 1]);
+      bf16x8 o;
+#pragma unroll
+      for (int q = 0; q < 4; ++q) {
+        o[q] = (bf16)fmaxf(a0[q], 0.1f * a0[q]);
+        o[4 + q] = (bf16)fmaxf(a1[q], 0.1f * a1[q]);
+      }
+      if (c1_planar) *reinterpret_cast<bf16x8*>(c1 + ((((size_t)oy0 + oy) * 8 + 4 * p + lq) * OH + ox) * 8) = o;
+      else *reinterpret_cast<bf16x8*>(c1 + (prow0 + pix) * 64 + 32 * p + 8 * lq) = o;
+    }
+  }
+}
+
+}
diff --git a/few-shot-vit_amd/csrc/stem_pipe.hip b/few-shot-vit_amd/csrc/stem_pipe.hip
--- /dev/null
+++ b/few-shot-vit_amd/csrc/stem_pipe.hip
@@ -0,0 +1,105 @@
+#include "kernels.h"
+#include "stem_conv1.h"
+#define FSVIT_HALO_DEVICE_ONLY
+#include "conv3x3_halo.hip"
+
+namespace FSVIT_NS {
+
+namespace stem_pipe {
+constexpr int P0 = stem1::OH * stem1::OH;
+constexpr size_t C1_BYTES = (size_t)P0 * 64 * 2, C2_BYTES = (size_t)P0 * 128 * 2, PAT_BYTES = (size_t)P0 * 32 * 2;
+constexpr size_t SCRATCH = C1_BYTES + C2_BYTES + PAT_BYTES;
+constexpr int GRID = 256;
+constexpr int TILE_ALLOC = (stem1::TILE_BYTES + 255) & ~255;
+constexpr int TILES = stem1::OH / halo::TR;
+static_assert(SCRATCH % 256 == 0 && 2 * TILE_ALLOC <= halo::OFF_W, "scratch regions stay 256-byte aligned; conv1's windows fit the halo buffers");
+}
+
+struct StemPipeParams {
+  const float* x;
+  const float* x2;
+  int B1, B;
+  const bf16* w1;
+  int kw1;
+  const float* b1;
+  ConvGemmParams p2, p3;
+  unsigned char* scratch;
+};
+
+__device__ __forceinline__ void stem_pipe_handoff(const int wave) {
+  asm volatile("s_waitcnt vmcnt(0)" ::: "memory");
+  __syncthreads();
+  if (wave == 0) {
+    __builtin_amdgcn_fence(__ATOMIC_ACQUIRE, "agent");
+    asm volatile("s_waitcnt vmcnt(0)" ::: "memory");
+  }
+  __syncthreads();
+}
+
+__device__ __forceinline__ int opaque(int v) {
+  asm volatile("" : "+v"(v));
+  return v;
+}
+
+__global__ __launch_bounds__(512, 2) void stem_pipe_kernel(const StemPipeParams q) {
+  using namespace stem_pipe;
+  extern __shared__ __attribute__((aligned(16))) unsigned char smem[];
+  const int t = threadIdx.x, lane = t & 63;
+  const int wave = __builtin_amdgcn_readfirstlane(t >> 6);
+  unsigned char* const sc = q.scratch + (size_t)blockIdx.x * SCRATCH;
+  bf16* const c1 = reinterpret_cast<bf16*>(sc);
+  bf16* const c2 = reinterpret_cast<bf16*>(sc + C1_BYTES);
+  bf16* const pat = reinterpret_cast<bf16*>(sc + C1_BYTES + C2_BYTES);
+  ConvGemmParams p2 = q.p2, p3 = q.p3;
+  p2.x = c1; p2.y = c2;
+  p3.x = c2; p3.x2 = pat;
+  const size_t x_img = (size_t)3 * stem1::IMG * stem1::IMG, x1_img = (size_t)(P0 / 4) * 128;
+  const int grp = wave >> 2, gw = wave & 3, tg = t & (stem1::NW * 64 - 1);
+  bf16* const tile = reinterpret_cast<bf16*>(smem + grp * TILE_ALLOC);
+
+#pragma unroll 1
+  for (int img = blockIdx.x; img < q.B; img += (int)gridDim.x) {
+    {
+      const float* xb = img < q.B1 ? q.x + (size_t)img * x_img : q.x2 + (size_t)(img - q.B1) * x_img;
+      const StemConv1Weights cw = stem_conv1_weights(q.w1, q.kw1, q.b1, opaque(lane));
+#pragma unroll 1
+      for (int r = 0; r < (TILES + 1) / 2; ++r) {
+        const int strip = 2 * r + grp;
+        if (r) __syncthreads();
+        if (strip < TILES) stem_conv1_stage(xb, tile, strip, tg);
+        __syncthreads();
+        if (strip < TILES) stem_conv1_tiles(tile, pat, c1, cw, strip, gw, lane, 1);
+      }
+    }
+    stem_pipe_handoff(wave);
+    conv3x3_halo_tiles<64, false>(p2, TILES, 0, []() { return 1; }, opaque(t));
+    stem_pipe_handoff(wave);
+    p3.y = reinterpret_cast<bf16*>(q.p3.y) + (size_t)img * x1_img;
+    conv3x3_halo_tiles<128, true>(p3, TILES, 0, []() { return 1; }, opaque(t));
+    __syncthreads();
+  }
+}
+
+bool stem_pipe_supported(int dtype, int img, int C0, int C1) { return dtype == 1 && img == stem1::IMG && C0 == 64 && C1 == 128; }
+size_t stem_pipe_scratch_bytes() { return stem_pipe::SCRATCH; }
+int stem_pipe_grid() { return stem_pipe::GRID; }
+
+int launch_stem_pipe(const float* x, const float* x2, int B1, int B, const void* w1, int kw1, const float* b1, const ConvGemmParams& p2, const ConvGemmParams& p3,
+                     void* scratch, int grid, hipStream_t s) {
+  if (B <= 0) return 0;
+  if (!conv3x3_halo_eligible(p2, 1) || !conv3x3_halo_eligible(p3, 1) || p2.B != 1 || p3.B != 1 || p2.H != stem1::OH || p3.H != stem1::OH || p2.Cin != 64 ||
+      p2.pool2 || p2.stats || p2.w_cpad || !p2.x_planar || !p2.y_planar || !p3.pool2 || p3.w_cpad || !p3.x_planar || p3.x2_cstride != 32 || B1 < 0 || B1 > B ||
+      (B1 < B && !x2) || grid <= 0)
+    return (int)hipErrorInvalidValue;
+  hipError_t e = hipFuncSetAttribute((const void*)stem_pipe_kernel, hipFuncAttributeMaxDynamicSharedMemorySize, halo::LDS_BYTES);
+  if (e != hipSuccess) return (int)e;
+  StemPipeParams q;
+  q.x = x; q.x2 = x2; q.B1 = B1; q.B = B;
+  q.w1 = (const bf16*)w1; q.kw1 = kw1; q.b1 = b1;
+  q.p2 = p2; q.p3 = p3;
+  q.scratch = (unsigned char*)scratch;
+  hipLaunchKernelGGL(stem_pipe_kernel, dim3(grid < B ? grid : B), dim3(512), halo::LDS_BYTES, s, q);
+  return (int)hipGetLastError();
+}
+
+}
diff --git a/few-shot-vit_amd/engine.py b/few-shot-vit_amd/engine.py
--- a/few-shot-vit_amd/engine.py
+++ b/few-shot-vit_amd/engine.py
@@ -730,6 +730,23 @@
             _lib.check(lib.fsvit_stem_conv1_dt(_ptr(x.contiguous()), _ptr(w), w.shape[-1], _ptr(bias), _ptr(patches), _ptr(c1), B, H, W, dt,
                                                _stream_ptr(x.device)))
         return patches, c1
+
+    @staticmethod
+    def stem_pipe(x, w1, b1, w2, b2, w3, b3, pos, x2=None, grid=0, scratch=None):
+        _require_cuda(x, w1, w2, w3, pos)
+        dt = ops._dt16(w1)
+        lib = _lib.load()
+        B1 = x.shape[0]
+        B = B1 + (x2.shape[0] if x2 is not None else 0)
+        g = grid if grid > 0 else lib.fsvit_stem_pipe_grid()
+        if scratch is None:
+            scratch = torch.empty(min(g, B) * lib.fsvit_stem_pipe_scratch_bytes(), dtype=torch.uint8, device=x.device)
+        x1 = torch.empty(B, 20, 20, 128, dtype=w1.dtype, device=x.device)
+        with torch.cuda.device(x.device):
+            _lib.check(lib.fsvit_stem_pipe(_ptr(x.contiguous()), _ptr(x2.contiguous()) if x2 is not None else None, B1, B, _ptr(w1), w1.shape[-1], _ptr(b1),
+                                           _ptr(w2), w2.shape[-1], _ptr(b2), _ptr(w3), w3.shape[-1], _ptr(b3), _ptr(pos), _ptr(scratch), _ptr(x1), int(grid),
+                                           dt, _stream_ptr(x.device)))
+        return x1
 
     @staticmethod
     def maxpool2_pos(x, pos):
diff --git a/include/fsvit.h b/include/fsvit.h
--- a/include/fsvit.h
+++ b/include/fsvit.h
@@ -47,6 +47,7 @@
 int fsvit_visformer_out_dim(const fsvit_visformer* h);
 int fsvit_visformer_dtype(const fsvit_visformer* h);
 size_t fsvit_visformer_workspace_bytes(const fsvit_visformer* h, int chunk_images);
+size_t fsvit_visformer_plan_bytes(const fsvit_visformer_cfg* cfg, int dtype, int chunk_images);
 int fsvit_visformer_forward(fsvit_visformer* h, const float* x_nchw_dev, int n_img, int img_h, int img_w,
                             float* feat_dev, void* ws_dev, size_t ws_bytes, void* stream);
 int fsvit_encoder_set_tap(void* encoder, const char* name, void* dst_dev, size_t bytes);
@@ -158,6 +159,11 @@
                                   int heads, int hdp, float eps, float scale, int dtype, void* stream);
 int fsvit_stem_conv1_dt(const float* x_nchw_dev, const void* w_dev, int kw, const float* bias_dev, void* patches_dev, void* c1_dev,
                         int B, int H, int W, int dtype, void* stream);
+size_t fsvit_stem_pipe_scratch_bytes(void);
+int fsvit_stem_pipe_grid(void);
+int fsvit_stem_pipe(const float* x_nchw_dev, const float* xsrc2_dev, int B1, int B, const void* w1_dev, int kw1, const float* b1_dev, const void* w2_dev,
+                    int kw2, const float* b2_dev, const void* w3_dev, int kw3, const float* b3_dev, const float* pos_dev, void* scratch_dev, void* x1_dev,
+                    int grid, int dtype, void* stream);
 int fsvit_visformer_last_tokens(fsvit_visformer* h, const void* ws_dev, size_t ws_bytes, int n_img, float* tokens_dev, void* stream);
 int fsvit_linear_forward(const float* x_dev, const float* w_dev, const float* b_dev, float* y_dev, int M, int N, int K, void* stream);
 int fsvit_linear_backward(const float* dy_dev, const float* x_dev, const float* w_dev, float* dx_dev, int accumulate_dx, float* dw_dev,
```

Measured after the change: 4503 episodes/s (median of 6 runs). About the same (+0.3%).
